# kieranrcampbell/clonealign

Hardware: AMD Instinct MI355X
Metric: ELBO iterations/sec (higher is better)
Workload: dtype f32 variables (contraction: float64 series over gene bins; count-matrix products: int8 MFMA, exact); 1 GPU; synthetic 100000 cells x 5000 genes x 8 clones, K=1, S=1, cell-sharded over 1 GPU(s) (BASELINE.json configs[2]); cells=100000, genes=5000, clones=8, K=1, mc_samples=1, y_storage=u8, y_bytes_per_elem=1, fused_sweep=True, fwd_mfma=True, series_form=True, y_mfma=True, parallelism=single, collective=none, allreduce_doubles_per_train_pass=20764, build_id=f943299e0af595e5

## Files before the change

### clonealign_amd/csrc/ca_eng_create.inc

```

constexpr double CA_ML_STREAM_FIXED_US = 6.6;
constexpr double CA_ML_STREAM_BYTES_PER_US = 5.62e6;
constexpr double CA_ML_MIN_STREAM_US = 45.0;
constexpr int CA_ML_MAX_PER = 4;
struct ca_mom_last_in {
  int slots;
  int n_cu;
  int nb_stream, nb_ovf;
  int ngrp, nred;
  int64_t image_bytes;
};
inline int ca_mom_last_free(const ca_mom_last_in& a) { return std::max(a.slots - a.nb_stream, 0); }
inline int ca_mom_last_free_x(const ca_mom_last_in& a) {
  const int xcd = std::max(a.n_cu / 32, 1);
  return a.slots / xcd - cdiv(a.nb_stream, xcd);
}
inline int ca_mom_last_per(const ca_mom_last_in& a) {
  const int xcd = std::max(a.n_cu / 32, 1), free_x = ca_mom_last_free_x(a);
  if (free_x < 1) return 0;
  return std::max(1, cdiv(a.ngrp, free_x * xcd));
}
inline bool ca_mom_last_pick(const ca_mom_last_in& a) {
  if (a.nb_stream + a.ngrp + a.nred <= a.slots) return false;
  const int per = ca_mom_last_per(a);
  if (per < 1 || per > CA_ML_MAX_PER) return false;
  return CA_ML_STREAM_FIXED_US + (double)a.image_bytes / CA_ML_STREAM_BYTES_PER_US >= CA_ML_MIN_STREAM_US;
}

int create_impl(ca_engine* h, const ca_problem* p) {
  const int N = (int)h->N; (void)N;
  HIPCK(h, hipSetDevice(h->device));
  hipDeviceProp_t prop;
  HIPCK(h, hipGetDeviceProperties(&prop, h->device));
  h->n_cu = prop.multiProcessorCount > 0 ? prop.multiProcessorCount : 256;
  HIPCK(h, hipStreamCreateWithFlags(&h->stream, hipStreamNonBlocking));
  HIPCK(h, hipStreamCreateWithFlags(&h->stream2, hipStreamNonBlocking));
  HIPCK(h, hipEventCreateWithFlags(&h->ev_params, hipEventDisableTiming));
  HIPCK(h, hipEventCreateWithFlags(&h->ev_ydone, hipEventDisableTiming));
  {
    int lo = 0, hi = 0;
    if (hipDeviceGetStreamPriorityRange(&lo, &hi) != hipSuccess) { (void)hipGetLastError(); lo = hi = 0; }
    if (hipStreamCreateWithPriority(&h->stream3, hipStreamNonBlocking, hi) != hipSuccess) { (void)hipGetLastError(); h->stream3 = nullptr; }
  }
  HIPCK(h, hipEventCreateWithFlags(&h->ev_poly0, hipEventDisableTiming));
  HIPCK(h, hipEventCreateWithFlags(&h->ev_poly1, hipEventDisableTiming));
  HIPCK(h, hipEventCreateWithFlags(&h->ev_ywdone, hipEventDisableTiming));
  h->async_y = variant_on(h, CA_VAR_ASYNC_Y, "CA_ASYNC_Y") &&
               ((double)h->N * (double)h->G >= 4e7 || variantx_on(h, CA_VARX_ASYNC_SMALL, "CA_ASYNC_SMALL"));
  HIPCK(h, hipHostMalloc((void**)&h->host_pinned, 64 * sizeof(double)));
  memset(h->host_pinned, 0, 64 * sizeof(double));
  if (hipHostGetDevicePointer((void**)&h->host_dev, h->host_pinned, 0) != hipSuccess) { h->host_dev = nullptr; (void)hipGetLastError(); }
  h->mon_tail = no_small_args();
  h->tail_fuse = variant_on(h, CA_VAR_TAIL_FUSE, "CA_TAIL_FUSE");
  h->pre_ok = variant_on(h, CA_VAR_PRE, "CA_PRE");
  h->upd_merge = h->tail_fuse && h->pre_ok && variant_on(h, CA_VAR_UPDATE_MERGE, "CA_UPDATE_MERGE");
  h->p2p_ride = h->tail_fuse && variant_on(h, CA_VAR_P2P_RIDE, "CA_P2P_RIDE");
  h->run_gate = h->upd_merge && variant_on(h, CA_VAR_RUN_GATE, "CA_RUN_GATE");
  {
    int khz = 0;
    if (hipDeviceGetAttribute(&khz, hipDeviceAttributeWallClockRate, h->device) == hipSuccess && khz >= 1000) h->ticks_per_us = (double)khz / 1000.0;
    else (void)hipGetLastError();
  }
  h->gate_ticks = (unsigned long long)(h->ticks_per_us * (double)(h->opt.gate_timeout_us > 0 ? h->opt.gate_timeout_us : 1000));
  h->run_fwd = h->run_gate && variantx_on(h, CA_VARX_RUN_FWD, "CA_RUN_FWD");
  h->pair_elbo = variant_on(h, CA_VAR_PAIR_ELBO, "CA_PAIR_ELBO");
  CACK(h->sp_in ? upload_y_sparse(h, p, h->sp_in) : upload_y(h, p));
  const int G = h->G, C = h->C, K = h->K, P = h->P, S = h->S, D = h->D;
  const int64_t Nn = h->N;
  h->nchunk = cdiv(C, CA_CW);
  h->ngblk = cdiv(G, CA_TB);
  {
    int CP = 1;
    while (CP < C) CP <<= 1;
    h->ncblk = (C <= 64) ? std::min(cdiv(Nn, CA_TB / CP), 16 * 256) : cdiv(Nn, CA_TB);
  }
  const int target_blocks = 8 * h->n_cu;
  const int nfb = cdiv(Nn, CA_TB * kFwdR);
  h->gsplit = std::max(1, std::min(std::min(target_blocks / std::max(nfb, 1), 16), std::max(1, G / 64)));
  h->gsplit = std::max(h->gsplit, cdiv(G, 1024));
  if (const int t = tune_val(h, CA_TUNE_GSPLIT, "CA_GSPLIT")) h->gsplit = std::max(std::max(1, t), cdiv(G, 1024));
  h->gchunk = cdiv(G, h->gsplit);
  h->gsplit = cdiv(G, h->gchunk);
  h->RG = G >= 1024 ? 4 : 1;
  if (const int r = tune_val(h, CA_TUNE_RG, "CA_RG")) { if (r == 1 || r == 4 || r == 8) h->RG = r; }
  h->ntile = cdiv(G, 64 * h->RG);
  const int gblocks = cdiv(h->ntile, CA_TB / 64);
  h->csplit = (int)std::max<int64_t>(1, std::min<int64_t>(cdiv(target_blocks, gblocks), std::max<int64_t>(1, Nn / 64)));
  if (const int t = tune_val(h, CA_TUNE_CSPLIT, "CA_CSPLIT")) h->csplit = std::max(1, t);
  h->cchunk = (Nn + h->csplit - 1) / h->csplit;
  h->csplit = cdiv(Nn, h->cchunk);
  h->TR = 128;
  const int tr_set = tune_val(h, CA_TUNE_TR, "CA_TR");
  if (tr_set) h->TR = std::min(128, std::max(1, tr_set));
  h->nrb = cdiv(Nn, h->TR);
  while (!tr_set && (int64_t)h->nrb * h->nseg < 4 * h->n_cu && h->TR > 32) { h->TR /= 2; h->nrb = cdiv(Nn, h->TR); }
  h->nrg = cdiv(h->nrb, CA_TB / 64);
  std::vector<double> Lrm((size_t)G * C), logL((size_t)G * C);
  std::vector<float> Lb((size_t)(h->nchunk + (h->nchunk & 1)) * G * CA_CW, 0.f);
  for (int g = 0; g < G; ++g)
    for (int c = 0; c < C; ++c) {
      const double v = p->L[hidx(p->layout, g, c, G, C)];
      Lrm[(size_t)g * C + c] = v;
      logL[(size_t)g * C + c] = std::log(v);
      Lb[((size_t)(c / CA_CW) * G + g) * CA_CW + (c % CA_CW)] = (float)v;
    }
  CACK(dalloc(h, &h->Lb, (int64_t)Lb.size()));
  CACK(upload_f(h, h->Lb, Lb));
  double* logL_dev = nullptr; double* extra_dev = nullptr;
  HIPCK(h, hipMalloc((void**)&logL_dev, logL.size() * sizeof(double)));
// ... 145 lines not shown
    }
    int zsplit = h->gsplit;
    if (h->fwd_mfma) {
      h->frow = 16;
      h->nk32 = cdiv(G, 32);
      const int cblocks = cdiv(Nn, (CA_TB / 64) * CA_FM_TL * 16);
      {
        int per_cu = 4;
        const void* fn = (D == 1) ? (const void*)k_fwd_mfma<1> : (const void*)k_fwd_mfma<2>;
        if (hipOccupancyMaxActiveBlocksPerMultiprocessor(&per_cu, fn, CA_TB, 0) != hipSuccess || per_cu < 1) per_cu = 4;
        (void)hipGetLastError();
        h->fsplit = pick_split(cblocks, (int64_t)per_cu * h->n_cu, std::max(1, std::min(16, h->nk32 / CA_FM_KC)), 0.02);
      }
      if (const int t = tune_val(h, CA_TUNE_FSPLIT, "CA_FSPLIT")) h->fsplit = std::max(1, std::min(t, h->nk32));
      h->fkchunk = cdiv(h->nk32, h->fsplit);
      h->fsplit = cdiv(h->nk32, h->fkchunk);
      zsplit = h->fsplit;
      CACK(dalloc(h, &h->Mq, (int64_t)h->nk32 * 2 * 64 * 8 * ((h->c16 || h->s2) ? 2 : 1)));
    } else {
      CACK(dalloc(h, &h->Mb2, (int64_t)G * h->frow));
    }
    CACK(dalloc(h, &h->mu32B, G));
    CACK(dalloc(h, &h->gene_partB, (int64_t)h->ngblk * (3 + K)));
    CACK(dalloc(h, &h->gene_part_alt, (int64_t)h->ngblk * (3 + K)));
    CACK(dalloc(h, &h->gene_partB_alt, (int64_t)h->ngblk * (3 + K)));
    if (!h->fwd_cell) CACK(dalloc(h, &h->Zpart2, (int64_t)zsplit * Nn * h->frow));
  }
  if (!h->fwd_cell) h->async_y = false;
  if (verbose(h))
    fprintf(stderr, "[clonealign_hip] N=%lld G=%d C=%d D=%d n_cu=%d gsplit=%d gchunk=%d csplit=%d fused=%d fwd_mfma=%d fsplit=%d fkchunk=%d "
            "bwd_mfma=%d csplit_m=%d cchunk_m=%lld nwt=%d fwd_cell=%d fc_tl=%d fc_nbig=%d ncblk_f=%d ystore=%d async_y=%d\n", (long long)Nn, G, C, D, h->n_cu, h->gsplit,
            h->gchunk, h->csplit, (int)h->fused_ok, (int)h->fwd_mfma, h->fsplit, h->fkchunk, (int)h->bwd_mfma, h->csplit_m,
            (long long)h->cchunk_m, h->nwt, (int)h->fwd_cell, h->fc_tl, h->fc_nbig, h->ncblk_f, h->ystore, (int)h->async_y);
  CACK(dalloc(h, &h->vmm, 2 * std::max(D, 1)));
  CACK(dalloc(h, &h->vmm_part, (int64_t)h->ngblk * 2 * std::max(D, 1)));
  CACK(dalloc(h, &h->etamax2, h->N16));
  CACK(dalloc(h, &h->gene_part, (int64_t)h->ngblk * (3 + K)));
  CACK(dalloc(h, &h->Zpart, (int64_t)S * h->gsplit * h->nchunk * Nn * CA_CW));
  CACK(dalloc(h, &h->coef, (int64_t)S * h->nchunk * Nn * CA_CW));
  CACK(dalloc(h, &h->scratch, Nn * C));
  const int64_t n_cpart = std::max(std::max(h->ncblk, h->ncblk_f), h->n_cu);
  CACK(dalloc(h, &h->cell_part, n_cpart * (3 + C)));
#ifdef CA_SERIES_ALWAYS
  const bool series_auto = true;
#else
  const bool series_auto = Nn >= 6000 && (double)G >= 2000.0 + (h->opt.world > 1 ? 7.5e7 : 2.5e7) / (double)Nn;
#endif
  h->adam_bound = ca_adam_step_bound(h->opt.learning_rate, h->opt.beta1, h->opt.beta2);
  h->poly_shape = ca_poly_ok(D, S, C) && h->fused_ok && !h->c16 && !h->s2 && K == 1 && h->adam_bound > 0 &&
                  (variant_on(h, CA_VAR_SERIES, "CA_SERIES") || variantx_on(h, CA_VARX_SERIES, "CA_SERIES_ON"));
  h->poly = h->poly_shape && ((series_auto && variant_on(h, CA_VAR_SERIES, "CA_SERIES")) || variantx_on(h, CA_VARX_SERIES, "CA_SERIES_ON"));
  if (h->poly) {
    int CPp = 1;
    while (CPp < C) CPp <<= 1;
    const int per_cu = (h->opt.reserved[0] >= 1 && h->opt.reserved[0] <= 8) ? h->opt.reserved[0] : 2;
    const int ncb = (int)std::min<int64_t>(cdiv(Nn, CA_TB / CPp), (int64_t)per_cu * h->n_cu);
    h->poly_side = h->opt.reserved[1] == 1;
    const size_t wb = ca_poly_workspace_bytes(G, ncb);
    CACK(dalloc(h, &h->poly_mem, (int64_t)wb));
    HIPCK(h, hipMemsetAsync(h->poly_mem, 0, wb, h->stream));
    ca_poly_bind(&h->pws, h->poly_mem, G, ncb);
    HIPCK(h, hipHostMalloc((void**)&h->poly_ring, 16 * 4 * sizeof(double), hipHostMallocMapped));
    memset(h->poly_ring, 0, 16 * 4 * sizeof(double));
    if (hipHostGetDevicePointer((void**)&h->poly_ring_dev, h->poly_ring, 0) != hipSuccess) { (void)hipGetLastError(); h->poly = false; }
    CACK(dalloc(h, &h->poly_xpart, cdiv(Nn, CA_TB)));
    CACK(dalloc(h, &h->poly_zero, Nn));
    HIPCK(h, hipMemsetAsync(h->poly_zero, 0, (size_t)Nn * sizeof(float), h->stream));
  }
  CACK(dalloc(h, &h->ee_partB, n_cpart));
  CACK(dalloc(h, &h->gpart, (int64_t)std::max(h->csplit, h->csplit_m) * G * (S + D)));
  CACK(dalloc(h, &h->dFpart, (int64_t)std::max(h->ntile, h->nwt) * Nn * std::max(D, 1)));
  CACK(dalloc(h, &h->YWpart, (int64_t)(h->nseg + 1) * Nn * std::max(K, 1)));
  CACK(dalloc(h, &h->YTpart, (int64_t)(h->nrb + 1) * h->Gp * std::max(K, 1)));
  CACK(dalloc(h, &h->YW, Nn * std::max(K, 1)));
  h->n_yw = cdiv(Nn, CA_TB);
  CACK(dalloc(h, &h->yw_part, h->n_yw));
  CACK(dalloc(h, &h->ytpsi, (int64_t)h->Gp * std::max(K, 1)));
  if (h->ystore == CA_YSTORE_U8 && K == 1 && h->Gp < (1 << 21) && Nn < ((int64_t)1 << 26) && variant_on(h, CA_VAR_Y_MFMA1, "CA_Y_MFMA1")) {
    h->ys_N64 = (Nn + 63) / 64 * 64;
    h->ys_nseg = h->Gp / CA_YS_GW;
    h->ys_RS = 64;
    while (h->ys_RS < 512 && cdiv(Nn, 4 * h->ys_RS) * h->ys_nseg > 4 * h->n_cu) h->ys_RS *= 2;
    h->ys_nrg = cdiv(Nn, 4 * h->ys_RS);
    const bool y4_force = variantx_on(h, CA_VARX_Y4, "CA_Y4_ON");
    if (variant_on(h, CA_VAR_Y4, "CA_Y4") && (h->poly || y4_force) && (double)Nn * (double)h->Gp < 2.0e9) {
      const int64_t nkeys = (int64_t)h->ys_nrg * h->ys_nseg * 4 * h->ys_RS;
      CACK(dalloc(h, &h->esc_off, nkeys + 1));
      const int64_t nw = Nn * h->ys_nseg;
      hipLaunchKernelGGL(k_esc_count, dim3(cdiv(nw * 64, CA_YM_TB)), dim3(CA_YM_TB), 0, h->stream, (const uint8_t*)h->Y, Nn, h->Gp, h->ys_nseg, h->ys_RS,
                         h->esc_off);
      hipLaunchKernelGGL(k_esc_scan, dim3(1), dim3(1024), 0, h->stream, h->esc_off, nkeys);
      HIPCK(h, hipGetLastError());
      int total = 0;
      HIPCK(h, hipMemcpyAsync(&total, h->esc_off + nkeys, sizeof(int), hipMemcpyDeviceToHost, h->stream));
      SYNC(h);
      h->n_esc = total;
      h->ys4 = h->n_esc * 256 <= Nn * (int64_t)h->G || y4_force;
      if (!h->ys4) {
        HIPCK(h, hipFree(h->esc_off));
        h->allocs.pop_back();
        h->dev_bytes -= 4 * (nkeys + 1);
        h->esc_off = nullptr;
      } else {
        CACK(dalloc(h, &h->esc, h->n_esc));
        hipLaunchKernelGGL(k_esc_fill, dim3(cdiv(nw * 64, CA_YM_TB)), dim3(CA_YM_TB), 0, h->stream, (const uint8_t*)h->Y, Nn, h->Gp, h->ys_nseg, h->ys_RS,
                           h->esc_off, h->esc);
        HIPCK(h, hipGetLastError());
      }
    }
    CACK(dalloc(h, &h->Ys, h->ys_N64 * h->Gp / (h->ys4 ? 2 : 1)));
    uint8_t *wr = nullptr, *pr = nullptr;
    CACK(dalloc(h, &wr, (int64_t)(h->Gp / 64) * 1024));
    CACK(dalloc(h, &pr, (h->ys_N64 / 64) * 1024));
    h->Wr = (uint4*)wr; h->Pr = (uint4*)pr;
    CACK(dalloc(h, &h->Wsum, (int64_t)(h->Gp / 64) * 4));
    CACK(dalloc(h, &h->Psum, (h->ys_N64 / 64) * 4));
    CACK(dalloc(h, &h->YWpart, (int64_t)(std::max(h->nseg, h->ys_nseg) + 1) * Nn));
    CACK(dalloc(h, &h->YTpart, (int64_t)(std::max(h->nrb, h->ys_nrg) + 1) * h->Gp));
    CACK(dalloc(h, &h->ys_exps, 6));
    CACK(dalloc(h, &h->ys_amax, 2));
    h->ys_nq = cdiv((int64_t)(h->Gp / 64) + h->ys_N64 / 64, CA_YM_TB / 64);
    h->ys_ncap = std::max(h->ys_nq, h->ngblk + cdiv(Nn, CA_TB)) + 2;
    CACK(dalloc(h, &h->ys_amaxp, (int64_t)3 * h->ys_ncap * 2));
    if (h->ys4)
      hipLaunchKernelGGL(k_pack_y4, dim3(cdiv(h->ys_N64 * (h->Gp / 32), CA_YM_TB)), dim3(CA_YM_TB), 0, h->stream, (const uint8_t*)h->Y, (uint4*)h->Ys, Nn,
                         h->ys_N64, h->Gp);
    else
      hipLaunchKernelGGL(k_bias_y, dim3(cdiv(h->ys_N64 * (h->Gp / 16), CA_YM_TB)), dim3(CA_YM_TB), 0, h->stream, (const uint8_t*)h->Y, (uint4*)h->Ys, Nn,
                         h->ys_N64, h->Gp);
    HIPCK(h, hipGetLastError());
    if (h->adam_bound > 0) h->ys_step_bound = (float)(1.02 * h->adam_bound);
    h->y_ys = true;
    h->y_dev_bytes += h->ys4 ? h->ys_N64 * h->Gp / 2 + 4 * h->n_esc + 4 * ((int64_t)h->ys_nrg * h->ys_nseg * 4 * h->ys_RS + 1) : h->ys_N64 * h->Gp;
  }
  h->mom_ride = h->poly && h->y_ys && !h->poly_side && h->host_dev && variant_on(h, CA_VAR_MOM_RIDE, "CA_MOM_RIDE");
  if (h->mom_ride) {
    ca_mom_last_in ml;
    int per_cu = 0;
    const hipError_t oe = h->ys4 ? (h->n_ovf > 0 ? hipOccupancyMaxActiveBlocksPerMultiprocessor(&per_cu, k_ys_mfma_ovf_mom<true>, CA_YM_TB, CA_YS4_LDS_BYTES)
                                                 : hipOccupancyMaxActiveBlocksPerMultiprocessor(&per_cu, k_ys_mfma_mom<true>, CA_YM_TB, CA_YS4_LDS_BYTES))
                                 : (h->n_ovf > 0 ? hipOccupancyMaxActiveBlocksPerMultiprocessor(&per_cu, k_ys_mfma_ovf_mom<false>, CA_YM_TB, CA_YS_LDS_BYTES)
                                                 : hipOccupancyMaxActiveBlocksPerMultiprocessor(&per_cu, k_ys_mfma_mom<false>, CA_YM_TB, CA_YS_LDS_BYTES));
    if (oe != hipSuccess) { (void)hipGetLastError(); per_cu = 0; }
    ml.slots = per_cu * h->n_cu; ml.n_cu = h->n_cu;
    ml.nb_stream = h->ys_nrg * h->ys_nseg;
    ml.nb_ovf = h->n_ovf > 0 ? cdiv(Nn, CA_TB) + cdiv(h->n_ovf_chunk, CA_TB / 64) : 0;
    ml.ngrp = h->pws.n_gene_blocks; ml.nred = CA_MOM_NRED;
    ml.image_bytes = h->ys_N64 * h->Gp / (h->ys4 ? 2 : 1);
    h->mom_free_slots = ca_mom_last_free(ml);
    h->mom_last = variantx_on(h, CA_VARX_MOM_LAST, "CA_MOM_LAST_ON") || (variant_on(h, CA_VAR_MOM_LAST, "CA_MOM_LAST") && ca_mom_last_pick(ml));
    if (h->opt.variant_off & CA_VAR_MOM_LAST) h->mom_last = false;
    if (h->mom_last) {
      const int per = ca_mom_last_per(ml);
      h->mom_per = per < 1 ? CA_MOM_PER : std::min(per, CA_ML_MAX_PER);
      h->mom_nred = 2 * CA_MOM_NRED;
      const int lab = (h->opt.reserved[1] & ~0xFF) ? h->opt.reserved[1] >> 8 : 0;
      if (lab & 15) h->mom_per = lab & 15;
      if (lab & 16) h->mom_nred = CA_MOM_NRED;
      h->mom_ovf_first = (lab & 32) != 0;
    }
  }
  h->cell_lean = h->poly && variant_on(h, CA_VAR_CELL_LEAN, "CA_CELL_LEAN");
  h->cell_mfma = h->poly && variant_on(h, CA_VAR_CELL_MFMA, "CA_CELL_MFMA");
  h->ride_ok = h->ystore == CA_YSTORE_U8 && K == 1 && D <= 2 && h->fused_ok && !h->c16 && h->fwd_cell && (h->fc_tl == 6 || h->fc_tl == 8 || (h->fc_tl == 2 && h->fc_nbig == 0)) &&
               !h->y_ys && variant_on(h, CA_VAR_Y_RIDE, "CA_Y_RIDE");
  const bool tl1_ok = h->fc_tl == 1 && h->fc_nbig == 0 && !h->c16;
  h->ride_ys = h->y_ys && (!h->ys4 || (h->poly && D == 1 && !h->c16 && !h->s2)) && D <= 2 && h->fused_ok && h->fwd_cell && (h->fc_tl == 6 || tl1_ok || (h->fc_tl == 2 && h->fc_nbig == 0)) &&
               variant_on(h, CA_VAR_Y_RIDE, "CA_Y_RIDE");
  h->yfin_split = h->ride_ys && h->bwd_mfma && h->tail_fuse && variant_on(h, CA_VAR_YFIN_RIDE, "CA_YFIN_RIDE");
  if (h->y_ys && !h->ride_ys) h->async_y = false;
  {
    const int tiles = cdiv(Nn, 16), qb = tiles / std::max(h->n_cu, 1), rb = tiles - qb * h->n_cu;
    h->fwd_bal = h->ride_ys && !h->c16 && !h->s2 && D == 1 && C <= 8 && qb >= 1 && qb <= 6 && h->nk32 >= 96 && h->host_dev && variant_on(h, CA_VAR_FWD_BAL, "CA_FWD_BAL");
    if (h->fwd_bal) {
      h->bal_q = qb; h->bal_r = rb;
      h->bal_nchunk = rb > 0 ? std::min(CA_BAL_MAXCHUNK, h->n_cu / rb) : 0;
      CACK(dalloc(h, &h->bal_xw, std::max<int64_t>(1, (int64_t)rb * h->bal_nchunk * 512)));
    }
  }
  h->s2f = h->s2 && h->fused_ok && h->fwd_cell && (h->fc_tl == 2 || h->fc_tl == 6) && (h->ride_ys || !h->ride_ok) && variant_on(h, CA_VAR_S2_FUSE, "CA_S2_FUSE");
  h->layout_series = h->poly || (h->poly_shape && h->opt.world > 1);
  if (h->layout_series) {
    h->off_y = 3 + C;
    h->off_q = h->off_y + (int64_t)h->Gp * K;
    h->off_x = h->off_q + (int64_t)CA_PL_NB * (CA_PL_R + 2) * 8;
    h->off_g = h->off_x + std::max(h->opt.world, 1);
    h->red_n = h->off_g + (int64_t)G * (S + D);
    CACK(dalloc(h, &h->red, h->red_n));
    if (h->poly) h->pws.tabQ = h->red + h->off_q;
  } else {
  h->off_g = 3 + C;
  h->off_y = h->off_g + (int64_t)G * (S + D);
  h->red_n = h->off_y + (int64_t)G * K;
  CACK(dalloc(h, &h->red, h->off_y + (int64_t)h->Gp * std::max(K, 1)));
  }
  CACK(dalloc(h, &h->terms_dev, 4));
  CACK(ensure_elbo_cap(h, 64));
  CACK(ensure_eps_cap(h, 1));
  {
    const int cols = 1 + ((K > 0) ? P : 0);
    const int cols_all = cols + (p->loc0 ? 0 : 1);
    std::vector<double> srow;
    if (!p->loc0) {
      srow.resize((size_t)Nn);
      HIPCK(h, hipMemcpyAsync(srow.data(), h->s64, (size_t)Nn * sizeof(double), hipMemcpyDeviceToHost, h->stream));
      SYNC(h);
    }
    std::vector<double> cs((size_t)G, 0.0), ytx((size_t)G * std::max(P, 1), 0.0);
    float *Ft = nullptr, *Vt = nullptr, *YWp = nullptr, *YTp = nullptr; double* yt = nullptr;
    HIPCK(h, hipMalloc((void**)&Ft, (size_t)Nn * sizeof(float)));
    HIPCK(h, hipMalloc((void**)&Vt, (size_t)G * sizeof(float)));
    HIPCK(h, hipMalloc((void**)&YWp, (size_t)h->nseg * Nn * sizeof(float)));
    HIPCK(h, hipMalloc((void**)&YTp, (size_t)h->nrb * h->Gp * sizeof(float)));
// ... 66 lines not shown
```

### clonealign_amd/csrc/ca_eng_loop.inc

```
int wait_y(ca_engine* h, bool all) {
  if (all) {
    if (h->y_pending) HIPCK(h, hipStreamWaitEvent(h->stream, h->ev_ydone, 0));
    h->y_pending = false; h->yw_pending = false;
  } else if (h->yw_pending) {
    HIPCK(h, hipStreamWaitEvent(h->stream, h->ev_ywdone, 0));
    h->yw_pending = false;
  }
  return CA_OK;
}

int make_etamax(ca_engine* h) {
  if (h->D > 0) {
    LAUNCH(h, CA_KERNEL_OTHER, hipLaunchKernelGGL(k_vmm_final, dim3(1), dim3(64), 0, h->stream, h->vmm_part, h->vmm, h->ngblk, h->D));
    LAUNCH(h, CA_KERNEL_OTHER, hipLaunchKernelGGL(k_etamax, dim3(cdiv(h->N, CA_TB)), dim3(CA_TB), 0, h->stream, h->F, h->vmm, h->etamax2, h->N, h->D));
  }
  h->em_stale = false;
  return CA_OK;
}
int ensure_etamax(ca_engine* h) {
  if (!h->em_stale) return CA_OK;
  return make_etamax(h);
}

int refresh_derived(ca_engine* h) {
  CACK(wait_y(h, true));
  h->y_defer = false;
  h->pre_valid = false;
  h->ys_steps = -1;
  h->ys_quant_ready = false;
  if (h->D > 0) LAUNCH(h, CA_KERNEL_OTHER, hipLaunchKernelGGL(k_vprep, dim3(h->ngblk), dim3(CA_TB), 0, h->stream, h->V, h->Vs, h->vmm_part, h->G, h->D));
  CACK(make_etamax(h));
  h->gaux_slot = -1;
  h->ycache_valid = false;
  h->yfin_pending = false;
  h->look_valid = false;
  h->poly_fresh = false;
  h->poly_seq_base = h->poly_seq + 1;
  h->poly_xmax_ready = false;
  h->poly_xglob_steps = -1;
  return CA_OK;
}

ca_ovf_args ovf_args(ca_engine* h, float* YWextra) {
  ca_ovf_args ovf;
  memset(&ovf, 0, sizeof(ovf));
  if (h->n_ovf > 0) {
    ovf.nb_rows = cdiv(h->N, CA_TB); ovf.nb_chunks = cdiv(h->n_ovf_chunk, CA_TB / 64);
    ovf.rowptr = h->ovf_rowptr; ovf.col = h->ovf_col; ovf.val = h->ovf_val; ovf.YWextra = YWextra;
    ovf.chunk_start = h->ovf_chunk_start; ovf.row2 = h->ovf_row2; ovf.val2 = h->ovf_val2; ovf.csum = h->ovf_csum; ovf.nchunk = h->n_ovf_chunk;
  }
  return ovf;
}
ca_yfin_args yfin_args(ca_engine* h, int rows, int nseg) {
  ca_yfin_args a;
  memset(&a, 0, sizeof(a));
  a.ncol = cdiv((int64_t)h->Gp * h->K, 64); a.nrow = h->n_yw;
  a.part = h->YTpart; a.out = h->red + h->off_y; a.rows = rows; a.ld = (int64_t)h->Gp * h->K; a.cols = h->Gp * h->K; a.G = h->G;
  if (h->n_ovf > 0) { a.col_chunk_ptr = h->ovf_col_chunk_ptr; a.csum = h->ovf_csum; }
  a.YWpart = h->YWpart; a.nseg = nseg + (h->n_ovf > 0 ? 1 : 0); a.F = h->F; a.D = h->D; a.N = h->N; a.YW = h->YW; a.yw_part = h->yw_part;
  return a;
}
int launch_yfinish(ca_engine* h, int rows, int nseg) {
  const ca_yfin_args a = yfin_args(h, rows, nseg);
  LAUNCH(h, CA_KERNEL_OTHER, hipLaunchKernelGGL(k_yfinish, dim3(a.ncol + a.nrow), dim3(1024), 0, h->stream, a.part, a.out, a.rows, a.ld, a.cols, a.col_chunk_ptr,
                                                a.csum, h->K, a.G, a.ncol, a.YWpart, a.nseg, a.F, a.D, a.N, a.YW, a.yw_part));
  return CA_OK;
}

ca_ysq_args ys_quant_args(ca_engine* h, int steps, bool* lagged) {
  ca_ysq_args a;
  memset(&a, 0, sizeof(a));
  const int s0 = h->ys_slot, s1 = (s0 + 1) % 3;
  a.nblk = h->ys_nq;
  a.V = h->V; a.Dv = h->D; a.G = h->G; a.GS = h->Gp / 64; a.F = h->F; a.Df = h->D; a.N = h->N; a.NS = h->ys_N64 / 64;
  *lagged = steps >= 0 && steps <= 4 && h->ys_step_bound > 0.f;
  if (*lagged) {
    a.amax_in = h->ys_amaxp + (int64_t)s0 * h->ys_ncap * 2; a.n_in = h->ys_namax[s0];
    a.slack_w = a.slack_p = (float)steps * h->ys_step_bound;
  } else {
    a.amax_in = reinterpret_cast<const float*>(h->ys_amax); a.n_in = 1;
  }
  a.amax_out = h->ys_amaxp + (int64_t)s1 * h->ys_ncap * 2;
  h->ys_namax[s1] = h->ys_nq;
  a.exps = h->ys_exps + 2 * s0; a.Wr = h->Wr; a.Pr = h->Pr; a.Wsum = h->Wsum; a.Psum = h->Psum;
  return a;
}
int ys_quant(ca_engine* h) {
  if (h->ys_quant_ready) return CA_OK;
  bool lagged = false;
  ca_ysq_args a = ys_quant_args(h, h->ys_steps, &lagged);
  if (!lagged) {
    HIPCK(h, hipMemsetAsync(h->ys_amax, 0, 2 * sizeof(unsigned), h->stream));
    LAUNCH(h, CA_KERNEL_OTHER, hipLaunchKernelGGL(k_ym_absmax, dim3(cdiv(std::max<int64_t>(h->N, h->G), CA_YM_TB)), dim3(CA_YM_TB), 0, h->stream,
                                                  h->V, h->D, (int64_t)h->G, h->F, h->D, h->N, 1, h->ys_amax));
  }
  LAUNCH(h, CA_KERNEL_OTHER, hipLaunchKernelGGL(k_ys_quant, dim3(a.nblk), dim3(CA_YM_TB), 0, h->stream, a));
  return CA_OK;
}
ca_ys_io ys_io(ca_engine* h) {
  ca_ys_io io;
  io.Wr = h->Wr; io.Pr = h->Pr; io.Wsum = h->Wsum; io.Psum = h->Psum; io.exps = h->ys_exps + 2 * h->ys_slot;
  io.YWpart = h->YWpart; io.YTpart = h->YTpart;
  io.esc_off = h->ys4 ? h->esc_off : nullptr; io.esc = h->ys4 ? h->esc : nullptr;
  return io;
}
ca_ovf_args ys_ovf(ca_engine* h) { return ovf_args(h, h->YWpart + (int64_t)h->ys_nseg * h->N); }
int yfin_flush(ca_engine* h) {
  if (!h->yfin_pending) return CA_OK;
  h->yfin_pending = false;
  return launch_yfinish(h, h->ys_nrg, h->ys_nseg);
}
int ys_finish(ca_engine* h, bool defer = false) {
  h->yfin_pending = true;
  if (!defer) CACK(yfin_flush(h));
  h->ys_slot = (h->ys_slot + 1) % 3;
  h->ys_steps = 0;
  h->ys_quant_ready = false;
  h->ycache_valid = true;
  return CA_OK;
}
template <bool Y4>
void launch_ys(ca_engine* h) {
  constexpr int lds = Y4 ? CA_YS4_LDS_BYTES : CA_YS_LDS_BYTES;
  const int nb_main = h->ys_nrg * h->ys_nseg;
  const ca_pm_args* pm = h->mom_args;
  h->mom_args = nullptr;
  const int nmom = pm ? pm->nmb + pm->nred : 0;
  if (h->n_ovf > 0) {
    const ca_ovf_args ovf = ys_ovf(h);
    const dim3 grid(nmom + nb_main + ovf.nb_rows + ovf.nb_chunks);
    if (pm) {
      ca_pm_args pmo = *pm;
      if (h->mom_last && h->mom_ovf_first) pmo.blk0 += ovf.nb_rows + ovf.nb_chunks;
      hipLaunchKernelGGL(k_ys_mfma_ovf_mom<Y4>, grid, dim3(CA_YM_TB), lds, h->stream, h->Ys, ys_io(h), h->N, h->Gp, h->ys_RS, nb_main, ovf, h->F, h->V, h->D, pmo);
    }
    else hipLaunchKernelGGL(k_ys_mfma_ovf<Y4>, grid, dim3(CA_YM_TB), lds, h->stream, h->Ys, ys_io(h), h->N, h->Gp, h->ys_RS, nb_main, ovf, h->F, h->V, h->D);
  } else {
    if (pm) hipLaunchKernelGGL(k_ys_mfma_mom<Y4>, dim3(nmom + nb_main), dim3(CA_YM_TB), lds, h->stream, h->Ys, ys_io(h), h->N, h->Gp, h->ys_RS, *pm);
    else hipLaunchKernelGGL(k_ys_mfma<Y4>, dim3(nb_main), dim3(CA_YM_TB), lds, h->stream, h->Ys, ys_io(h), h->N, h->Gp, h->ys_RS);
  }
}
int ycache_ys(ca_engine* h) {
  CACK(ys_quant(h));
  if (h->ys4) LAUNCH(h, CA_KERNEL_YPASS, launch_ys<true>(h));
  else LAUNCH(h, CA_KERNEL_YPASS, launch_ys<false>(h));
  const bool defer = h->ys_defer_next;
  h->ys_defer_next = false;
  return ys_finish(h, defer);
}

int ensure_ycache(ca_engine* h) {
  if (h->y_defer) {
    h->y_defer = false;
    HIPCK(h, hipStreamWaitEvent(h->stream2, h->ev_params, 0));
    std::swap(h->stream, h->stream2);
    h->on_side = true;
    const int rc = ensure_ycache(h);
    h->on_side = false;
    std::swap(h->stream, h->stream2);
    CACK(rc);
    HIPCK(h, hipEventRecord(h->ev_ydone, h->stream2));
    h->y_pending = true;
    HIPCK(h, hipEventRecord(h->ev_ywdone, h->stream2));
    h->yw_pending = true;
    return CA_OK;
  }
  if (h->ycache_valid || h->K == 0) { h->ycache_valid = true; return yfin_flush(h); }
  h->yfin_pending = false;
  if (h->y_ys) return ycache_ys(h);
  dim3 grid((unsigned)((int64_t)h->nrg * h->nseg));
  const ca_ovf_args ovf = ovf_args(h, h->YWpart + (int64_t)h->nseg * h->N * h->K);
  ca_ovf_args none;
  memset(&none, 0, sizeof(none));
  const ca_ypass_ops fit = {h->F, h->D, h->V, h->YWpart, h->YTpart, h->K};
  for (int koff = 0; koff < h->K; koff += 4) {
    const int kk = std::min(4, h->K - koff);
    CACK(prof_begin(h, CA_KERNEL_YPASS));
    const ca_ovf_args& o = koff == 0 ? ovf : none;
    ypass<0>(h, fit, koff, kk, grid, o);
    HIPCK(h, hipGetLastError());
    CACK(prof_end(h));
  }
  if (!h->on_side) {
    CACK(launch_yfinish(h, h->nrg, h->nseg));
  } else {
    LAUNCH(h, CA_KERNEL_OTHER, hipLaunchKernelGGL(k_colsum, dim3(cdiv((int64_t)h->Gp * h->K, 64)), dim3(1024), 0, h->stream,
                                                  h->YTpart, h->red + h->off_y, h->nrg, (int64_t)h->Gp * h->K, h->Gp * h->K,
                                                  h->n_ovf > 0 ? h->ovf_col_chunk_ptr : nullptr, h->n_ovf > 0 ? h->ovf_csum : nullptr, h->K, h->G));
    LAUNCH(h, CA_KERNEL_OTHER, hipLaunchKernelGGL(k_yw_dot, dim3(h->n_yw), dim3(CA_TB), 0, h->stream, h->YWpart,
                                                  h->nseg + (h->n_ovf > 0 ? 1 : 0), h->F, h->D, h->K, h->N, h->YW, h->yw_part));
  }
  h->ycache_valid = true;
  return CA_OK;
}


ca_small_args small_args(ca_engine* h, const double* gene_part, int apply, float lr_t, double* elbo_dst, bool reduce_cells) {
  ca_small_args a;
  a.enabled = 1;
  a.red = h->red; a.gene_part = gene_part; a.ngblk = h->ngblk;
  a.vchi = h->vchi; a.alpha_u = h->alpha_u; a.m_v = h->m_v; a.v_v = h->v_v; a.m_a = h->m_a; a.v_a = h->v_a; a.g_v = h->g_v; a.g_a = h->g_a;
  a.elbo_out = elbo_dst; a.terms_out = h->terms_dev;
  a.G = h->G; a.C = h->C; a.K = h->K; a.apply = apply;
  a.lr_t = lr_t; a.b1 = (float)h->opt.beta1; a.b2 = (float)h->opt.beta2; a.aeps = (float)h->opt.adam_eps;
  a.vmm_part = h->vmm_part; a.vmm = h->vmm; a.D = h->D;
  a.dir_const = h->dir_const;
  a.cell_part = reduce_cells ? h->cell_part : nullptr; a.ncblk = h->ncblk;
  a.host_out = nullptr; a.host_flag = nullptr; a.host_seq = 0; a.reduce_only = 0;
  a.yw_part = nullptr; a.n_yw = 0;
  a.ee_part = nullptr; a.n_ee = 0;
  a.vchi_out = nullptr; a.alpha_out = nullptr;
  if (!apply && elbo_dst && h->host_seq_next && h->host_dev) {
    a.host_out = h->host_dev + 32;
    a.host_flag = reinterpret_cast<unsigned long long*>(h->host_dev + 33);
    a.host_seq = h->host_seq_next;
    h->host_seq_next = 0;
  }
  return a;
}
int mon_tail_local_sums(ca_engine* h) {
  if (!h->mon_tail.enabled || !h->mon_tail.cell_part) return CA_OK;
  CACK(wait_y(h, false));
  ca_small_args r = h->mon_tail;
  r.reduce_only = 1; r.host_out = nullptr;
  LAUNCH(h, CA_KERNEL_OTHER, hipLaunchKernelGGL(k_final_small, dim3(1), dim3(CA_TB), 0, h->stream, r));
  h->mon_tail.cell_part = nullptr; h->mon_tail.yw_part = nullptr;
  return CA_OK;
// ... 753 lines not shown
```

### clonealign_amd/csrc/ca_eng_state.inc

```
namespace {

thread_local std::string g_last_error;

typedef struct { char internal[128]; } ca_nccl_uid;
typedef void* ca_nccl_comm;
struct RcclApi {
  void* lib = nullptr;
  int (*GetUniqueId)(ca_nccl_uid*) = nullptr;
  int (*CommInitRank)(ca_nccl_comm*, int, ca_nccl_uid, int) = nullptr;
  int (*CommDestroy)(ca_nccl_comm) = nullptr;
  int (*AllReduce)(const void*, void*, size_t, int, int, ca_nccl_comm, hipStream_t) = nullptr;
  const char* (*GetErrorString)(int) = nullptr;
  std::string err;
  bool load() {
    if (lib) return true;
    const char* cands[] = {getenv("CLONEALIGN_RCCL_LIB"), "librccl.so.1", "librccl.so", "/opt/rocm/lib/librccl.so.1",
                           "/opt/rocm/lib/librccl.so"};
    for (const char* c : cands) {
      if (!c || !*c) continue;
      lib = dlopen(c, RTLD_NOW | RTLD_LOCAL);
      if (lib) break;
    }
    if (!lib) { err = std::string("cannot dlopen librccl: ") + dlerror(); return false; }
    GetUniqueId = (decltype(GetUniqueId))dlsym(lib, "ncclGetUniqueId");
// ... 64 lines not shown
  const ca_sparse* sp_in = nullptr;
  float* Lb = nullptr;
  double *A = nullptr, *cn = nullptr, *s64 = nullptr, *colsum = nullptr, *YtX = nullptr;
  float* s32 = nullptr;
  float *F = nullptr, *m_psi = nullptr, *v_psi = nullptr;
  float *glogit = nullptr, *m_gl = nullptr, *v_gl = nullptr;
  float *V = nullptr, *m_V = nullptr, *v_V = nullptr;
  float *loc = nullptr, *ls = nullptr, *m_loc = nullptr, *v_loc = nullptr, *m_ls = nullptr, *v_ls = nullptr;
  float* loc_init = nullptr;
  float *vchi = nullptr, *m_v = nullptr, *v_v = nullptr;
  float *alpha_u = nullptr, *m_a = nullptr, *v_a = nullptr;
  float *vchi_alt = nullptr, *alpha_u_alt = nullptr;
  bool upd_merge = false, em_stale = false;
  bool run_gate = false, gate_req = false, gate_armed = false;
  unsigned long long gate_ticks = 100000ull; std::chrono::steady_clock::time_point gate_t0;
  double ticks_per_us = 100.0;
  bool gate_open = false, gate_aborted = false, in_run = false; struct gate_snapshot* gate_snap = nullptr; struct fwd_snapshot* gate_fsnap = nullptr;
  bool run_fwd = false;
  bool fwd_gate = false;
  unsigned long long gate_seq = 0; unsigned long long* gate_local = nullptr;
  bool p2p_ride = false;
  double* gaux = nullptr; int64_t gaux_slot = -1;
  int gaux_idx = 0;
  int* vmm_at = nullptr; int vmm_at_idx = 0; bool vmm_at_ready = false;
  double dir_const = 0.0;
  float b1p = 0.f, b2p = 0.f;
  float *g_loc = nullptr, *g_ls = nullptr, *g_V = nullptr, *g_v = nullptr, *g_a = nullptr, *g_psi = nullptr, *dgl = nullptr;
  float* eps_dev = nullptr; int64_t eps_cap = 0;
  float *mu32 = nullptr, *Mb = nullptr, *Vs = nullptr, *vmm = nullptr, *vmm_part = nullptr, *etamax2 = nullptr;
  double* gene_part = nullptr; int ngblk = 0;
  float *Zpart = nullptr, *coef = nullptr; double* scratch = nullptr;
  double* cell_part = nullptr; int ncblk = 0;
  float *gpart = nullptr, *dFpart = nullptr; int gsplit = 1, gchunk = 0, csplit = 1; int64_t cchunk = 0; int RG = 4, ntile = 0;
  float *YWpart = nullptr, *YTpart = nullptr, *YW = nullptr; double* ytpsi = nullptr;
  double* red = nullptr; int64_t red_n = 0, off_g = 0, off_y = 0;
  int64_t off_q = 0, off_x = 0;
  bool poly_shape = false, layout_series = false;
  bool mon_tail_local = false;
  bool poly_xslot_pending = false;
  int poly_xglob_steps = -1;
  double* elbo_dev = nullptr; int64_t elbo_cap = 0; double* terms_dev = nullptr;
  double* host_pinned = nullptr;
  bool ycache_valid = false, sums_global = false, sums_started = false;
  std::vector<double> mu_part;
  bool fused_ok = false, look_valid = false; int64_t look_slot = 0; int frow = 8;
  bool carry = false, carry_builtin = false; std::vector<float> carry_eps;
  int64_t n_series = 0, n_series_fallback = 0;
  double *poly_ring = nullptr, *poly_ring_dev = nullptr; uint64_t poly_seq = 0, poly_seq_base = 1, adam_steps = 0, poly_steps_at[16] = {};
  bool mom_ride = false; unsigned mom_tag = 0; const ca_pm_args* mom_args = nullptr;
  bool mom_last = false, mom_ovf_first = false; int mom_free_slots = 0, mom_per = CA_MOM_PER, mom_nred = CA_MOM_NRED;
  bool cell_mfma = false;
  bool cell_lean = false;
  bool poly = false, poly_side = false, poly_y_defer = false, poly_fresh = false, poly_df = false ; ca_poly_ws pws; float* poly_zero = nullptr; unsigned char* poly_mem = nullptr;
  float *Mb2 = nullptr, *mu32B = nullptr, *Zpart2 = nullptr; double* gene_partB = nullptr;
  bool y_defer = false;
  bool ride_ok = false;
  bool ride_ys = false;
  bool fold_gsum = false, fold_now = false;
  int64_t hint_A = -1, hint_B = -1, pre_A = -1, pre_B = -1;
  bool pre_valid = false, pre_ok = true, pair_elbo = true;
  double* ee_partB = nullptr;
  double *gene_part_alt = nullptr, *gene_partB_alt = nullptr;
  bool bwd_ready = false; int64_t bwd_slot = -1;
  double* yw_part = nullptr; int n_yw = 0;
  bool yfin_split = false, yfin_pending = false;
  ca_small_args mon_tail;
  bool tail_fuse = true;
  double* host_dev = nullptr;
  unsigned long long host_seq = 0, host_seq_next = 0;
  float* eps_stage = nullptr; size_t eps_stage_bytes = 0;
  hipEvent_t ev_stage = nullptr;
  bool fwd_cell = false; int ncblk_f = 0, fc_tl = 4;
  int fc_nbig = 0;
  bool fwd_mfma = false; int fsplit = 1, fkchunk = 1, nk32 = 1; unsigned short* Mq = nullptr;
  bool fwd_bal = false; int bal_q = 0, bal_r = 0, bal_nchunk = 0; unsigned long long* bal_xw = nullptr; unsigned bal_tag = 0;
  bool pfwd = false; int pf_npair = 0, pf_fsplit = 1, pf_kchunk = 1; unsigned short* pf_Mq = nullptr; float* pf_Z = nullptr;
  int bwd_pairs = 0;
  bool bwd_mfma = false, bwd_frac = false, c16 = false, s2 = false, s2f = false;
  unsigned short* coefq = nullptr; int64_t N16 = 0, cchunk_m = 0; int csplit_m = 1, nwt = 0;
  int bwd_tl = CA_BWD_TL;
  uint64_t draw = 0;
  hipEvent_t ev_ywdone = nullptr; bool yw_pending = false, on_side = false;
  bool y_ys = false, ys4 = false; int* esc_off = nullptr; unsigned* esc = nullptr; int64_t n_esc = 0;
  uint8_t* Ys = nullptr; uint4 *Wr = nullptr, *Pr = nullptr; int *Wsum = nullptr, *Psum = nullptr;
  int* ys_exps = nullptr;
  unsigned* ys_amax = nullptr;
  float* ys_amaxp = nullptr; int ys_nq = 0;
  int ys_ncap = 0, ys_namax[3] = {0, 0, 0};
  bool ys_quant_ready = false;
  int ys_slot = 0, ys_steps = -1, ys_RS = 256, ys_nrg = 0, ys_nseg = 0; int64_t ys_N64 = 0; float ys_step_bound = -1.f;
  double adam_bound = -1.0;
  ca_p2p* p2p = nullptr;
  ca_nccl_comm comm = nullptr;
  ca_host_allreduce_fn host_ar = nullptr; void* host_ar_user = nullptr; double* host_ar_buf = nullptr; int64_t host_ar_cap = 0;
  std::vector<EvPair> ev_pool; size_t ev_used = 0; bool prof_open = false;
  unsigned prof_seen[CA_KERNEL_COUNT] = {0, 0, 0, 0, 0};
  double k_ms[CA_KERNEL_COUNT] = {0}; int64_t k_n[CA_KERNEL_COUNT] = {0};
  int n_cu = 256;
};

namespace {

#define HIPCK(h, call)                                                                       \
  do {                                                                                       \
    hipError_t e_ = (call);                                                                  \
    if (e_ != hipSuccess) {                                                                  \
      (h)->err = std::string(#call) + ": " + hipGetErrorString(e_);                          \
      return CA_ERR_HIP;                                                                     \
    }                                                                                        \
  } while (0)

#define CACK(call)                \
  do {                            \
    int rc_ = (call);             \
    if (rc_ != CA_OK) return rc_; \
  } while (0)

int comm_check(ca_engine* h) {
  if (h->host_pinned && *reinterpret_cast<volatile unsigned int*>(h->host_pinned + 41) != 0u) {
    h->err = "a forward-sweep block gave up waiting for a chunk of a left-over tile (k_fwd_bal_ys); the engine's state is undefined";
    return CA_ERR_STATE;
  }
  if (h->host_pinned && *reinterpret_cast<volatile unsigned int*>(h->host_pinned + 43) != 0u) {
    h->err = "a reducer block of the series form's moment role gave up waiting for the moment blocks of its launch (k_ys_mfma_mom); the engine's state is undefined";
    return CA_ERR_STATE;
  }
  if (h->host_pinned && *reinterpret_cast<volatile unsigned int*>(h->host_pinned + 42) != 0u) {
    h->err = "the series form of the contraction (CA_VARX_SERIES) cannot cover this fit's exponent range: max|psi| (max W - min W) exceeds 4 x " +
             std::to_string(CA_PL_NB) + " bins' worth; the passes since are truncated -- start over without the series form";
    return CA_ERR_STATE;
  }
  if (h->p2p && h->p2p->err_host && *reinterpret_cast<volatile unsigned long long*>(h->p2p->err_host) != 0ull) {
    h->err = "peer-to-peer all-reduce #" + std::to_string(*reinterpret_cast<volatile unsigned long long*>(h->p2p->err_host)) +
             ": a peer's data did not arrive within the time limit (peer lost or out of step); this engine's transport is dead -- "
             "destroy the engine and start over in a fresh process";
    return CA_ERR_COMM;
  }
  return CA_OK;
}
#define SYNC(h)                                          \
  do {                                                   \
    HIPCK(h, hipStreamSynchronize((h)->stream));         \
    CACK(comm_check(h));                                 \
  } while (0)

template <typename T>
int dalloc(ca_engine* h, T** p, int64_t n) {
  if (n <= 0) n = 1;
  void* q = nullptr;
  hipError_t e = hipMalloc(&q, (size_t)n * sizeof(T));
  if (e != hipSuccess) {
    h->err = std::string("hipMalloc of ") + std::to_string(n * sizeof(T)) + " bytes: " + hipGetErrorString(e);
    return CA_ERR_NOMEM;
  }
  e = hipMemsetAsync(q, 0, (size_t)n * sizeof(T), h->stream);
  if (e == hipSuccess) e = hipStreamSynchronize(h->stream);
  if (e != hipSuccess) { h->err = hipGetErrorString(e); return CA_ERR_HIP; }
  h->allocs.push_back(q);
  h->dev_bytes += n * (int64_t)sizeof(T);
  *p = (T*)q;
  return CA_OK;
}

int prof_flush(ca_engine* h) {
  if (h->ev_used == 0) return CA_OK;
  SYNC(h);
// ... 227 lines not shown
```

### clonealign_amd/csrc/ca_kernels.hip.h

```cpp
#pragma once
#include <hip/hip_runtime.h>
#include <stdint.h>

#define CA_CW 8
#define CA_LOG2E_F 1.44269504088896340736f
#define CA_LN2 0.69314718055994530942
#define CA_LOG2PI 1.83787706640934548356
#define CA_TB 256

template <int CTRL, int ROW_MASK>
__device__ __forceinline__ float ca_dpp_pull(float v) {
  return __builtin_bit_cast(
      float, __builtin_amdgcn_update_dpp(0, __builtin_bit_cast(int, v), CTRL, ROW_MASK, 0xF, false));
}
__device__ __forceinline__ float ca_wave_sum_lane63(float v) {
  v += ca_dpp_pull<0xB1, 0xF>(v);
  v += ca_dpp_pull<0x4E, 0xF>(v);
  v += ca_dpp_pull<0x141, 0xF>(v);
  v += ca_dpp_pull<0x140, 0xF>(v);
  v += ca_dpp_pull<0x142, 0xA>(v);
  v += ca_dpp_pull<0x143, 0xC>(v);
  return v;
}

// ... 594 lines not shown
}

struct ca_p2p_args {
  double* const* peers;
  int rank, world;
  int64_t cap;
  unsigned long long seq;
  unsigned long long* err;
  unsigned int* err_local;
  unsigned long long timeout_ticks;
  const float* gpart; int nslice; int64_t fold_lo, fold_n;
  const double* yw_part; int n_yw; int64_t yw_index;
};
__device__ __forceinline__ unsigned long long* ca_p2p_entry(double* slab, int64_t cap, int world, int par, int src, int64_t i) {
  return reinterpret_cast<unsigned long long*>(slab) + 2 * ((((int64_t)par * world + src) * cap) + i);
}
#ifndef CA_P2P_LAB
#define CA_P2P_LAB 0
#endif
__global__ void __launch_bounds__(CA_TB) k_p2p_allreduce(double* __restrict__ buf, int64_t n, ca_p2p_args a) {
  __shared__ unsigned int bad;
  if (threadIdx.x == 0) bad = __hip_atomic_load(a.err_local, __ATOMIC_RELAXED, __HIP_MEMORY_SCOPE_AGENT) != 0u;
  __syncthreads();
  if (bad) return;
  const int par = (int)(a.seq & 1ull);
  const unsigned long long tag = (a.seq & 0xFFFFFFFFull) << 32;
  const int64_t i0 = (int64_t)blockIdx.x * CA_TB + threadIdx.x, stride = (int64_t)gridDim.x * CA_TB;
  double yw_sum = 0.0;
  if (a.yw_part && a.yw_index >= 0 && a.yw_index < n && (a.yw_index / CA_TB) % gridDim.x == blockIdx.x) {
    __shared__ double smy[CA_TB];
    double ya = 0.0;
    for (int b = threadIdx.x; b < a.n_yw; b += CA_TB) ya += a.yw_part[b];
    yw_sum = ca_block_sum(ya, smy);
  }
  double* mine = a.peers[a.rank];
  for (int64_t i = i0; i < n; i += stride) {
    double v;
    if (a.gpart && i >= a.fold_lo && i < a.fold_lo + a.fold_n) {
      v = 0.0;
      const float* gp = a.gpart + (i - a.fold_lo);
      for (int sp0 = 0; sp0 < a.nslice; sp0 += 8) {
        float t[8];
#pragma unroll
        for (int q = 0; q < 8; ++q) t[q] = gp[(int64_t)(sp0 + q < a.nslice ? sp0 + q : a.nslice - 1) * a.fold_n];
#pragma unroll
        for (int q = 0; q < 8; ++q) v += (sp0 + q < a.nslice) ? (double)t[q] : 0.0;
      }
    } else {
      v = buf[i];
    }
    if (a.yw_part && i == a.yw_index) v += yw_sum;
    const unsigned long long bits = (unsigned long long)__double_as_longlong(v);
    const unsigned long long w0 = (bits & 0xFFFFFFFFull) | tag, w1 = (bits >> 32) | tag;
    for (int p = 0; p < a.world; ++p) {
      unsigned long long* e = ca_p2p_entry(a.peers[p], a.cap, a.world, par, a.rank, i);
      __hip_atomic_store(e, w0, __ATOMIC_RELAXED, __HIP_MEMORY_SCOPE_SYSTEM);
      __hip_atomic_store(e + 1, w1, __ATOMIC_RELAXED, __HIP_MEMORY_SCOPE_SYSTEM);
    }
  }
  const unsigned long long t0 = __builtin_amdgcn_s_memrealtime();
  for (int64_t i = i0; i < n; i += stride) {
    double s = 0.0;
    for (int r = 0; r < a.world; ++r) {
      const unsigned long long* e = ca_p2p_entry(mine, a.cap, a.world, par, r, i);
      unsigned long long w0 = __hip_atomic_load(e, __ATOMIC_RELAXED, __HIP_MEMORY_SCOPE_SYSTEM);
      unsigned long long w1 = __hip_atomic_load(e + 1, __ATOMIC_RELAXED, __HIP_MEMORY_SCOPE_SYSTEM);
      while (((w0 ^ tag) >> 32) != 0ull || ((w1 ^ tag) >> 32) != 0ull) {
        if (__builtin_amdgcn_s_memrealtime() - t0 > a.timeout_ticks) {
          unsigned long long expect = 0ull;
          __hip_atomic_compare_exchange_strong(a.err, &expect, a.seq, __ATOMIC_RELAXED, __ATOMIC_RELAXED, __HIP_MEMORY_SCOPE_SYSTEM);
          __hip_atomic_store(a.err_local, 1u, __ATOMIC_RELAXED, __HIP_MEMORY_SCOPE_AGENT);
          return;
        }
        __builtin_amdgcn_s_sleep(1);
        w0 = __hip_atomic_load(e, __ATOMIC_RELAXED, __HIP_MEMORY_SCOPE_SYSTEM);
        w1 = __hip_atomic_load(e + 1, __ATOMIC_RELAXED, __HIP_MEMORY_SCOPE_SYSTEM);
      }
      s += __longlong_as_double((long long)((w0 & 0xFFFFFFFFull) | (w1 << 32)));
    }
    buf[i] = s;
  }
}

template <bool Y4>
__global__ void __launch_bounds__(CA_YM_TB, Y4 ? CA_YS4_WAVES : CA_YS_WAVES) k_ys_mfma_ovf(const uint8_t* __restrict__ Ys, ca_ys_io io, int64_t N, int Gp, int RS,
                                                                       int nb_main, ca_ovf_args ovf, const float* __restrict__ F,
                                                                       const float* __restrict__ V, int Dstride) {
  if ((int)blockIdx.x >= nb_main) {
    const int b = (int)blockIdx.x - nb_main;
    if (b < ovf.nb_rows) ca_ovf_rows_body(b, ovf.rowptr, ovf.col, ovf.val, V, Dstride, ovf.YWextra, N, 1, 0);
    else ca_ovf_chunks_body(b - ovf.nb_rows, ovf.chunk_start, ovf.row2, ovf.val2, F, Dstride, ovf.csum, ovf.nchunk, 1, 0);
    return;
  }
  extern __shared__ __attribute__((aligned(16))) unsigned char ca_ys_dyn[];
  ca_ys_mfma_body<Y4 ? CA_YS4_DEPTH : CA_YS_DEPTH, Y4, true>((int)blockIdx.x, Ys, io, N, Gp, RS, ca_ys_dyn);
}

#include "ca_polymom.hip.h"
static_assert(sizeof(ca_pm_lds) <= (size_t)CA_YS_LDS_BYTES && sizeof(ca_pm_lds) <= (size_t)CA_YS4_LDS_BYTES, "the moment role's tables fit the stream's dynamic LDS");
template <bool Y4>
__global__ void __launch_bounds__(CA_YM_TB, Y4 ? CA_YS4_WAVES : CA_YS_WAVES) k_ys_mfma_mom(const uint8_t* __restrict__ Ys, ca_ys_io io, int64_t N, int Gp, int RS, ca_pm_args pm) {
  extern __shared__ __attribute__((aligned(16))) unsigned char ca_ys_dyn[];
  const int nmom = pm.nmb + pm.nred, rb = (int)blockIdx.x - pm.blk0;
  if (rb >= 0 && rb < nmom) { ca_pm_ride_block<CA_YM_TB>(pm, rb, ca_ys_dyn); return; }
  ca_ys_mfma_body<Y4 ? CA_YS4_DEPTH : CA_YS_DEPTH, Y4, true>(rb < 0 ? (int)blockIdx.x : (int)blockIdx.x - nmom, Ys, io, N, Gp, RS, ca_ys_dyn);
}
template <bool Y4>
__global__ void __launch_bounds__(CA_YM_TB, Y4 ? CA_YS4_WAVES : CA_YS_WAVES) k_ys_mfma_ovf_mom(const uint8_t* __restrict__ Ys, ca_ys_io io, int64_t N, int Gp, int RS,
                                                                           int nb_main, ca_ovf_args ovf, const float* __restrict__ F,
                                                                           const float* __restrict__ V, int Dstride, ca_pm_args pm) {
  extern __shared__ __attribute__((aligned(16))) unsigned char ca_ys_dyn[];
  const int nmom = pm.nmb + pm.nred, rb = (int)blockIdx.x - pm.blk0;
  if (rb >= 0 && rb < nmom) { ca_pm_ride_block<CA_YM_TB>(pm, rb, ca_ys_dyn); return; }
  const int blk = rb < 0 ? (int)blockIdx.x : (int)blockIdx.x - nmom;
  if (blk >= nb_main) {
    const int b = blk - nb_main;
    if (b < ovf.nb_rows) ca_ovf_rows_body(b, ovf.rowptr, ovf.col, ovf.val, V, Dstride, ovf.YWextra, N, 1, 0);
    else ca_ovf_chunks_body(b - ovf.nb_rows, ovf.chunk_start, ovf.row2, ovf.val2, F, Dstride, ovf.csum, ovf.nchunk, 1, 0);
    return;
  }
  ca_ys_mfma_body<Y4 ? CA_YS4_DEPTH : CA_YS_DEPTH, Y4, true>(blk, Ys, io, N, Gp, RS, ca_ys_dyn);
}

struct ca_ysride_args {
  const uint8_t* Ys; ca_ys_io io;
  const float* F; const float* V; int Df;
  int Gp, RS, nb_main, nb_y;
  int pat_a, pat_b;
  int pers;
  ca_ovf_args ovf;
};
#ifndef CA_YS_RIDE_WAVES
#define CA_YS_RIDE_WAVES 4
#endif
template <int D, int TLB, int TLS, int DEPTH, bool C16 = false, bool S2F = false, bool Y4 = false>
__global__ void __launch_bounds__(CA_TB, (DEPTH == 1 && !C16 && !S2F) ? CA_YS_RIDE_WAVES : 3) k_fwd_cell_mix_ys(const float* __restrict__ F, const float* __restrict__ etamax2,
                                                           const float* __restrict__ Vs, const unsigned short* __restrict__ Mq,
                                                           ca_cell_ptrs p, const float* __restrict__ alpha_u,
                                                           double* __restrict__ cell_part, int64_t N, int C, int K, int nk, int nbig,
                                                           int nf, ca_ysride_args y) {
  constexpr size_t FW = sizeof(ca_f32x4) * 4 * TLB * 64 + sizeof(double) * (CA_TB + 64);
  constexpr size_t SM = FW > (size_t)CA_YS_LDS_BYTES ? FW : (size_t)CA_YS_LDS_BYTES;
  __shared__ __attribute__((aligned(16))) unsigned char smem[SM];
  if (p.gate) {
    if (*p.gate != p.gate_go) return;
  }
  int idx;
  bool sweep;
  if (y.pers > 0) {
    const int b = (int)blockIdx.x;
    sweep = b >= y.pers && b < y.pers + nf;
    idx = sweep ? b - y.pers : (b < y.pers ? b : y.nb_main + (b - y.pers - nf));
  } else {
    sweep = ca_ride_split((int)blockIdx.x, nf, y.nb_y, y.pat_a, y.pat_b, idx);
  }
  CA_LAB_BLOCK_T0();
#define CA_YS_LEAVE() CA_LAB_LEAVE(ca_ys_out)
  if (!sweep) {
    if (idx >= y.nb_main) {
      const int b = idx - y.nb_main;
      if (b < y.ovf.nb_rows) ca_ovf_rows_body(b, y.ovf.rowptr, y.ovf.col, y.ovf.val, y.V, y.Df, y.ovf.YWextra, N, 1, 0);
      else ca_ovf_chunks_body(b - y.ovf.nb_rows, y.ovf.chunk_start, y.ovf.row2, y.ovf.val2, y.F, y.Df, y.ovf.csum, y.ovf.nchunk, 1, 0);
      CA_YS_LEAVE();
    }
    CA_PRIO_STREAM();
    if (y.pers > 0) {
      for (int u = idx; u < y.nb_main; u += y.pers) {
        if (u != idx) __syncthreads();
        ca_ys_mfma_body<DEPTH, Y4>(u, y.Ys, y.io, N, y.Gp, y.RS, smem);
      }
    } else {
      ca_ys_mfma_body<DEPTH, Y4>(idx, y.Ys, y.io, N, y.Gp, y.RS, smem);
    }
    CA_YS_LEAVE();
  }
  {
    ca_f32x4* comb = reinterpret_cast<ca_f32x4*>(smem);
    double* sm = reinterpret_cast<double*>(smem + sizeof(ca_f32x4) * 4 * TLB * 64);
    double* la = sm + CA_TB;
    ca_log_softmax_alpha(alpha_u, C, la);
    if (nbig > 0 && idx >= nbig)
      ca_fwd_cell_body<D, TLS, C16, S2F>(F, etamax2, Vs, Mq, p, cell_part, N, C, K, nk, (int64_t)nbig * (TLB * 16) + (int64_t)(idx - nbig) * (TLS * 16), idx, comb, sm, la);
    else
      ca_fwd_cell_body<D, TLB, C16, S2F>(F, etamax2, Vs, Mq, p, cell_part, N, C, K, nk, (int64_t)idx * (TLB * 16), idx, comb, sm, la);
  }
#undef CA_YS_LEAVE
  CA_LAB_LABEL(ca_ys_out);
  CA_LAB_BLOCK_END(sweep ? (nbig > 0 && idx >= nbig ? 2 : 1) : 0, idx);
}

#include "ca_fwdbal.hip.h"
#include "ca_k_mse.hip.h"
#include "ca_k_loglik.hip.h"
#include "ca_k_blockll.hip.h"
#include "ca_k_pairll.hip.h"
#include "ca_k_dmll.hip.h"
#include "ca_k_project.hip.h"
#include "ca_k_simulate.hip.h"
#include "ca_k_predictive.hip.h"
#include "ca_k_logexpr.hip.h"
```

### clonealign_amd/csrc/ca_ymfma.hip.h

```cpp
#pragma once
#include <hip/hip_runtime.h>
#include <stdint.h>

typedef int ca_i32x4 __attribute__((ext_vector_type(4)));

#define CA_YM_TB 256

__device__ __forceinline__ int ca_fix_exp(float amax) { return amax > 0.f ? 29 - ilogbf(amax) : 0; }

__global__ void __launch_bounds__(CA_YM_TB) k_ym_absmax(const float* __restrict__ V, int Dv, int64_t G, const float* __restrict__ F, int Df,
                                                        int64_t N, int K, unsigned* __restrict__ amax) {
  const int64_t i = (int64_t)blockIdx.x * CA_YM_TB + threadIdx.x;
  float mw = 0.f, mp = 0.f;
  if (i < G) for (int k = 0; k < K; ++k) mw = fmaxf(mw, fabsf(V[i * Dv + k]));
  if (i < N) for (int k = 0; k < K; ++k) mp = fmaxf(mp, fabsf(F[i * Df + k]));
#pragma unroll
  for (int o = 32; o > 0; o >>= 1) { mw = fmaxf(mw, __shfl_xor(mw, o, 64)); mp = fmaxf(mp, __shfl_xor(mp, o, 64)); }
  if ((threadIdx.x & 63) == 0) {
    if (i < G + 64) atomicMax(amax, __float_as_uint(mw));
    if (i < N + 64) atomicMax(amax + 1, __float_as_uint(mp));
  }
}
__device__ __forceinline__ int ca_digit(int x, int p) {
  int d = 0;
#pragma unroll
  for (int i = 0; i <= 3; ++i) {
    d = (int)(signed char)(x & 0xFF);
    if (i == p) break;
    x = (x - d) >> 8;
  }
  return d;
}
__global__ void __launch_bounds__(CA_YM_TB) k_bias_y(const uint8_t* __restrict__ Y, uint4* __restrict__ Ys, int64_t N, int64_t N64, int Gp) {
  const int64_t i = (int64_t)blockIdx.x * CA_YM_TB + threadIdx.x;
  const int64_t per_piece = 256, nb = Gp / 64;
  if (i >= (N64 / 64) * nb * per_piece) return;
  const int c = (int)(i & 3), r = (int)((i >> 2) & 63);
  const int64_t piece = i >> 8;
  const int64_t cs = piece / nb, gb = piece - cs * nb;
  const int64_t n = cs * 64 + r;
  uint4 v = {0u, 0u, 0u, 0u};
  if (n < N) v = *reinterpret_cast<const uint4*>(Y + n * (int64_t)Gp + gb * 64 + 16 * c);
  v.x ^= 0x80808080u; v.y ^= 0x80808080u; v.z ^= 0x80808080u; v.w ^= 0x80808080u;
  Ys[i] = v;
}

__device__ __forceinline__ unsigned ca_nib4(unsigned lo, unsigned hi) {
  unsigned r = 0;
#pragma unroll
  for (int b = 0; b < 4; ++b) {
    const unsigned x = (lo >> (8 * b)) & 0xFFu, y = (hi >> (8 * b)) & 0xFFu;
    r |= ((x < 15u ? x : 15u) | ((y < 15u ? y : 15u) << 4)) << (8 * b);
  }
  return r;
}
__global__ void __launch_bounds__(CA_YM_TB) k_pack_y4(const uint8_t* __restrict__ Y, uint4* __restrict__ Y4, int64_t N, int64_t N64, int Gp) {
  const int64_t i = (int64_t)blockIdx.x * CA_YM_TB + threadIdx.x;
  const int64_t nb = Gp / 64;
  if (i >= (N64 / 64) * nb * 128) return;
  const int l = (int)(i & 63), ld = (int)((i >> 6) & 1);
  const int64_t piece = i >> 7, cs = piece / nb, gb = piece - cs * nb;
  const int64_t n0 = cs * 64 + 32 * ld + (l & 15), n1 = n0 + 16;
  const uint8_t* base = Y + gb * 64 + 16 * (l >> 4);
  uint4 a = {0u, 0u, 0u, 0u}, b = {0u, 0u, 0u, 0u};
  if (n0 < N) a = *reinterpret_cast<const uint4*>(base + n0 * (int64_t)Gp);
  if (n1 < N) b = *reinterpret_cast<const uint4*>(base + n1 * (int64_t)Gp);
  Y4[i] = (uint4){ca_nib4(a.x, b.x), ca_nib4(a.y, b.y), ca_nib4(a.z, b.z), ca_nib4(a.w, b.w)};
}
__device__ __forceinline__ int64_t ca_esc_key(int64_t n, int seg, int nseg, int RS) {
  const int64_t s = n / RS;
  return (((s >> 2) * nseg + seg) * 4 + (s & 3)) * RS + (n - s * RS);
}
__device__ __forceinline__ int ca_esc_count8(uint2 v) {
  int c = 0;
#pragma unroll
  for (int b = 0; b < 4; ++b) c += (((v.x >> (8 * b)) & 0xFFu) >= 15u) + (((v.y >> (8 * b)) & 0xFFu) >= 15u);
  return c;
}
__global__ void __launch_bounds__(CA_YM_TB) k_esc_count(const uint8_t* __restrict__ Y, int64_t N, int Gp, int nseg, int RS, int* __restrict__ off) {
  const int64_t w = ((int64_t)blockIdx.x * CA_YM_TB + threadIdx.x) >> 6;
  const int lane = threadIdx.x & 63;
  if (w >= N * nseg) return;
  const int64_t n = w / nseg;
  const int seg = (int)(w - n * nseg);
  int c = ca_esc_count8(*reinterpret_cast<const uint2*>(Y + n * (int64_t)Gp + seg * 512 + 8 * lane));
#pragma unroll
  for (int o = 32; o > 0; o >>= 1) c += __shfl_xor(c, o, 64);
  if (lane == 0) off[ca_esc_key(n, seg, nseg, RS)] = c;
}
__global__ void __launch_bounds__(1024) k_esc_scan(int* __restrict__ off, int64_t n) {
  __shared__ int64_t sm[1024];
  const int t = threadIdx.x;
  const int64_t chunk = (n + 1023) / 1024, a = t * chunk, b = (a + chunk < n) ? a + chunk : n;
  int64_t s = 0;
  for (int64_t i = a; i < b; ++i) s += off[i];
  sm[t] = s;
  __syncthreads();
  for (int o = 1; o < 1024; o <<= 1) {
    const int64_t v = t >= o ? sm[t - o] : 0;
    __syncthreads();
    sm[t] += v;
    __syncthreads();
  }
  int64_t run = sm[t] - s;
  for (int64_t i = a; i < b; ++i) { const int c = off[i]; off[i] = (int)run; run += c; }
  if (t == 1023) off[n] = (int)sm[1023];
}
__global__ void __launch_bounds__(CA_YM_TB) k_esc_fill(const uint8_t* __restrict__ Y, int64_t N, int Gp, int nseg, int RS, const int* __restrict__ off,
                                                       unsigned* __restrict__ esc) {
  const int64_t w = ((int64_t)blockIdx.x * CA_YM_TB + threadIdx.x) >> 6;
  const int lane = threadIdx.x & 63;
  if (w >= N * nseg) return;
  const int64_t n = w / nseg;
  const int seg = (int)(w - n * nseg);
  const uint2 v = *reinterpret_cast<const uint2*>(Y + n * (int64_t)Gp + seg * 512 + 8 * lane);
  const int c = ca_esc_count8(v);
  int x = c;
#pragma unroll
  for (int o = 1; o < 64; o <<= 1) { const int u = __shfl_up(x, o, 64); if (lane >= o) x += u; }
  int e = off[ca_esc_key(n, seg, nseg, RS)] + x - c;
  const unsigned cl = (unsigned)(n % RS);
#pragma unroll
  for (int b = 0; b < 8; ++b) {
    const unsigned y = ((b < 4 ? v.x : v.y) >> (8 * (b & 3))) & 0xFFu;
    if (y >= 15u) esc[e++] = cl | ((unsigned)(8 * lane + b) << 9) | ((y - 15u) << 18);
  }
}

__device__ __forceinline__ ca_i32x4 ca_mfma_i8(uint4 a, uint4 b, ca_i32x4 c) {
  return __builtin_amdgcn_mfma_i32_16x16x64_i8(__builtin_bit_cast(ca_i32x4, a), __builtin_bit_cast(ca_i32x4, b), c, 0, 0, 0);
}

constexpr int CA_YS_GW = 512;
static_assert(CA_YS_GW == 512, "k_ys_mfma's accumulator switch has eight cases");
constexpr int CA_YS_PITCH = 80;

__device__ __forceinline__ void ca_ds_read_tr_b8_x8(unsigned addr, uint2 (&lo)[4], uint2 (&hi)[4]) {
  asm volatile(
      "ds_read_b64_tr_b8 %0, %8\n\tds_read_b64_tr_b8 %4, %8 offset:640\n\t"
      "ds_read_b64_tr_b8 %1, %8 offset:16\n\tds_read_b64_tr_b8 %5, %8 offset:656\n\t"
      "ds_read_b64_tr_b8 %2, %8 offset:32\n\tds_read_b64_tr_b8 %6, %8 offset:672\n\t"
      "ds_read_b64_tr_b8 %3, %8 offset:48\n\tds_read_b64_tr_b8 %7, %8 offset:688\n\t"
      "s_waitcnt lgkmcnt(0)"
      : "=&v"(lo[0]), "=&v"(lo[1]), "=&v"(lo[2]), "=&v"(lo[3]), "=&v"(hi[0]), "=&v"(hi[1]), "=&v"(hi[2]), "=&v"(hi[3])
      : "v"(addr)
      : "memory");
}
__device__ __forceinline__ void ca_ds_read_tr_b8_x4(unsigned addr, uint2 (&lo)[2], uint2 (&hi)[2]) {
  asm volatile(
      "ds_read_b64_tr_b8 %0, %4\n\tds_read_b64_tr_b8 %2, %4 offset:640\n\t"
      "ds_read_b64_tr_b8 %1, %4 offset:16\n\tds_read_b64_tr_b8 %3, %4 offset:656\n\t"
      "s_waitcnt lgkmcnt(0)"
      : "=&v"(lo[0]), "=&v"(lo[1]), "=&v"(hi[0]), "=&v"(hi[1])
      : "v"(addr)
      : "memory");
}
static_assert(8 * CA_YS_PITCH == 640, "offsets in ca_ds_read_tr_b8_x8 / _x4 assume the 80-byte pitch");
__device__ __forceinline__ uint4 ca_and4(uint4 a, unsigned m) { return (uint4){a.x & m, a.y & m, a.z & m, a.w & m}; }

#ifndef CA_YS_DEPTH
#define CA_YS_DEPTH 2
#endif
#ifndef CA_YS_WAVES
#define CA_YS_WAVES 3
#endif
struct ca_ys_io {
  const uint4* Wr; const uint4* Pr; const int* Wsum; const int* Psum; const int* exps;
  float* YWpart; float* YTpart;
  const int* esc_off; const unsigned* esc;
};
#ifndef CA_YS4_DEPTH
#define CA_YS4_DEPTH 4
#endif
#ifndef CA_YS4_WAVES
#define CA_YS4_WAVES 4
#endif
constexpr int CA_YS4_OFF_W = 4 * 64 * CA_YS_PITCH;
constexpr int CA_YS4_OFF_ROW = CA_YS4_OFF_W + (CA_YS_GW / 64) * 1024;
constexpr int CA_YS4_OFF_PSI = CA_YS4_OFF_ROW + 4 * 64 * 8;
constexpr int CA_YS4_OFF_COL = 4 * (CA_YS_GW / 64) * 64 * 4 * 4;
constexpr int CA_YS4_LDS_BYTES = CA_YS4_OFF_COL + CA_YS_GW * 8;
static_assert(CA_YS4_OFF_PSI + 4 * 256 <= CA_YS4_OFF_COL, "the 4-bit launch's tables fit below its column-escape sums");
static_assert(4 * CA_YS4_LDS_BYTES <= 160 * 1024, "four blocks of the 4-bit launch per CU");
template <int DEPTH = CA_YS_DEPTH, bool Y4 = false, bool OWN = false>
__device__ __forceinline__ void ca_ys_mfma_body(int blk, const uint8_t* __restrict__ Ys, const ca_ys_io& io, int64_t N, int Gp,
                                                int RS ,
                                                unsigned char* ca_ys_lds ) {
  const uint4* __restrict__ Wr = io.Wr;
  const uint4* __restrict__ Pr = io.Pr;
  constexpr bool Y4L = Y4 && OWN;
  constexpr int NP = CA_YS_GW / 64;
  static_assert(NP % DEPTH == 0, "pieces per cell step must be a multiple of the pipeline depth");
  const int lane = threadIdx.x & 63, j = lane & 15, q = lane >> 4;
  const int wv = __builtin_amdgcn_readfirstlane((int)(threadIdx.x >> 6) & 3);
  const int nseg = Gp / CA_YS_GW;
  const int rg = blk / nseg, seg = blk - rg * nseg;
  unsigned char* my = ca_ys_lds + (size_t)wv * 64 * CA_YS_PITCH;
  const int64_t c0 = ((int64_t)rg * 4 + wv) * RS;
  const int64_t c1 = (c0 + RS < N) ? c0 + RS : N;
  const int g0 = seg * CA_YS_GW;
  const unsigned grp = (unsigned)(j >> 2);
  unsigned msk[4];
#pragma unroll
  for (int t = 0; t < 4; ++t) msk[t] = grp == (unsigned)t ? 0xFFFFFFFFu : 0u;
  ca_i32x4 acc_yt[NP];
#pragma unroll
  for (int a = 0; a < NP; ++a) acc_yt[a] = (ca_i32x4){0, 0, 0, 0};
  const int lrow = lane >> 2, lch = lane & 3;
  unsigned char* wr_dst = my + lrow * CA_YS_PITCH + 16 * lch;
  const unsigned char* rd_row = my + j * CA_YS_PITCH + 16 * q;
  const unsigned rd_tr = (unsigned)(size_t)my + (unsigned)((16 * q + (j >> 1)) * CA_YS_PITCH + 8 * (j & 1));
  constexpr int PB = Y4 ? 2048 : 4096, NL = PB / 1024;
  const uint8_t* src = Ys + ((c0 >> 6) * (int64_t)(Gp / 64) + (g0 >> 6)) * PB;
  const uint4* wsrc = Wr + (int64_t)(g0 >> 6) * 64;
  const unsigned voff = 16u * (unsigned)lane;
  uint4 R[DEPTH][NL], W[DEPTH];
  const int nsteps = c0 < c1 ? (int)((c1 - c0 + 63) / 64) : 0;
  typedef unsigned ca_v4u __attribute__((ext_vector_type(4)));
  const __amdgpu_buffer_rsrc_t ry = __builtin_amdgcn_make_buffer_rsrc(const_cast<uint8_t*>(src), 0, 0x7FFFFFFF, 0x00020000);
  const __amdgpu_buffer_rsrc_t rw = __builtin_amdgcn_make_buffer_rsrc(const_cast<uint4*>(wsrc), 0, NP * 1024, 0x00020000);
  const __amdgpu_buffer_rsrc_t rp = __builtin_amdgcn_make_buffer_rsrc(const_cast<uint4*>(Pr + (c0 >> 6) * 64), 0, 0x7FFFFFFF, 0x00020000);
  auto issue = [&](int slot, int st, int a, unsigned vo) {
    const int so = (st * (Gp / 64) + a) * PB;
#pragma unroll
    for (int i = 0; i < NL; ++i) {
      const ca_v4u v = __builtin_amdgcn_raw_buffer_load_b128(ry, (int)(vo + 1024u * (unsigned)i), so, 2 );
      R[slot][i] = (uint4){v.x, v.y, v.z, v.w};
    }
    if (!Y4L) {
      const ca_v4u w = __builtin_amdgcn_raw_buffer_load_b128(rw, (int)voff, a * 1024, 0);
      W[slot] = (uint4){w.x, w.y, w.z, w.w};
    }
  };
  uint4* wl = reinterpret_cast<uint4*>(ca_ys_lds + CA_YS4_OFF_W);
  unsigned long long* colesc = reinterpret_cast<unsigned long long*>(ca_ys_lds + CA_YS4_OFF_COL);
  uint4 wimg[2];
  int eoff = 0;
  if (Y4L) {
    wimg[0] = wsrc[threadIdx.x];
    wimg[1] = wsrc[threadIdx.x + CA_YM_TB];
    if (lane <= nsteps) eoff = io.esc_off[((int64_t)blk * 4 + wv) * RS + (64 * lane < RS ? 64 * lane : RS)];
  }
  uint4 pr_nx = {0u, 0u, 0u, 0u};
  if (nsteps > 0) {
    if (Y4L) {
      const ca_v4u pv = __builtin_amdgcn_raw_buffer_load_b128(rp, (int)voff, 0, 0);
      pr_nx = (uint4){pv.x, pv.y, pv.z, pv.w};
    }
#pragma unroll
    for (int d_ = 0; d_ < DEPTH; ++d_) issue(d_, 0, d_, voff);
  }
  if (Y4L) {
    static_assert(2 * CA_YM_TB == CA_YS_GW, "the block's threads hold the segment's W image and column sums in two halves");
    wl[threadIdx.x] = wimg[0];
    wl[threadIdx.x + CA_YM_TB] = wimg[1];
    colesc[threadIdx.x] = 0ull;
    colesc[threadIdx.x + CA_YM_TB] = 0ull;
    __syncthreads();
  }
  ca_i32x4 acc_yw[4];
  uint4 prm[4];
  int wtot[4] = {0, 0, 0, 0};
  if (!Y4) {
    const int* ws = io.Wsum + (g0 >> 6) * 4;
#pragma unroll
    for (int a = 0; a < NP; ++a)
#pragma unroll
      for (int p_ = 0; p_ < 4; ++p_) wtot[p_] += ws[a * 4 + p_];
  }
  const int e_w = io.exps[0];
  const int64_t kb = ((int64_t)blk * 4 + wv) * RS;
  unsigned long long* rowesc = reinterpret_cast<unsigned long long*>(ca_ys_lds + (Y4L ? CA_YS4_OFF_ROW : 4 * 64 * CA_YS_PITCH)) + wv * 64;
  unsigned char* psl = ca_ys_lds + CA_YS4_OFF_PSI + wv * 256;
  if (Y4) rowesc[lane] = 0ull;
  for (int st = 0; st < nsteps; ++st) {
    const int64_t cs = c0 + (int64_t)st * 64;
    const bool more = st + 1 < nsteps;
    uint4 pr;
    if (Y4L) {
      pr = pr_nx;
#pragma unroll
      for (int t = 0; t < 4; ++t) acc_yw[t] = (ca_i32x4){0, 0, 0, 0};
    } else {
      const ca_v4u pv = __builtin_amdgcn_raw_buffer_load_b128(rp, (int)voff, st * 1024, 0);
      pr = (uint4){pv.x, pv.y, pv.z, pv.w};
#pragma unroll
      for (int t = 0; t < 4; ++t) { acc_yw[t] = (ca_i32x4){0, 0, 0, 0}; if (!Y4L) prm[t] = ca_and4(pr, msk[t]); }
    }
    int e_lo = 0, e_hi = 0;
    unsigned en0 = 0u, en1 = 0u;
    if (Y4L) {
      e_lo = __builtin_amdgcn_readlane(eoff, st);
      e_hi = __builtin_amdgcn_readlane(eoff, st + 1);
      if (e_hi > e_lo) {
        en0 = io.esc[e_lo + lane < e_hi ? e_lo + lane : e_hi - 1];
        en1 = io.esc[e_lo + 64 + lane < e_hi ? e_lo + 64 + lane : e_hi - 1];
      }
    }
#pragma unroll
    for (int a = 0; a < NP; ++a) {
      const int slot = a % DEPTH;
      __builtin_amdgcn_sched_barrier(0);
      const uint4 wr = Y4L ? wl[a * 64 + lane] : W[slot];
      if (Y4) {
#pragma unroll
        for (int t = 0; t < 4; ++t) {
          const uint4 v = R[slot][t >> 1];
          const int sh = 4 * (t & 1);
          const uint4 av = ca_and4((uint4){v.x >> sh, v.y >> sh, v.z >> sh, v.w >> sh}, 0x0F0F0F0Fu);
          *reinterpret_cast<uint4*>(const_cast<unsigned char*>(rd_row) + 16 * t * CA_YS_PITCH) = av;
          acc_yw[t] = ca_mfma_i8(av, wr, acc_yw[t]);
        }
        if (a + DEPTH < NP) issue(slot, st, a + DEPTH, voff);
        else if (Y4L) {
          const unsigned vo = more ? voff : 0x80000000u + voff;
          if (a + DEPTH == NP) {
            const ca_v4u pv = __builtin_amdgcn_raw_buffer_load_b128(rp, (int)vo, (st + 1) * 1024, 0);
            pr_nx = (uint4){pv.x, pv.y, pv.z, pv.w};
          }
          issue(slot, st + 1, a + DEPTH - NP, vo);
        } else if (more) issue(slot, st + 1, a + DEPTH - NP, voff);
      } else {
#pragma unroll
        for (int i = 0; i < 4; ++i) *reinterpret_cast<uint4*>(wr_dst + 16 * i * CA_YS_PITCH) = R[slot][i];
        if (a + DEPTH < NP) issue(slot, st, a + DEPTH, voff);
        else if (more) issue(slot, st + 1, a + DEPTH - NP, voff);
#pragma unroll
        for (int t = 0; t < 4; ++t) {
          const uint4 av = *reinterpret_cast<const uint4*>(rd_row + 16 * t * CA_YS_PITCH);
          acc_yw[t] = ca_mfma_i8(av, wr, acc_yw[t]);
        }
      }
#pragma unroll
      for (int h2 = 0; h2 < 2; ++h2) {
        uint2 lo[2], hi[2];
        ca_ds_read_tr_b8_x4(rd_tr + 32u * (unsigned)h2, lo, hi);
#pragma unroll
        for (int t = 0; t < 2; ++t) {
          uint4 pa;
          if (Y4L) {
            unsigned g_ = grp;
            asm volatile("" : "+v"(g_));
            pa = ca_and4(pr, g_ == (unsigned)(2 * h2 + t) ? 0xFFFFFFFFu : 0u);
          } else {
            pa = prm[2 * h2 + t];
          }
          acc_yt[a] = ca_mfma_i8(pa, (uint4){lo[t].x, lo[t].y, hi[t].x, hi[t].y}, acc_yt[a]);
        }
      }
    }
    if (Y4L) {
      if (j < 4) *reinterpret_cast<uint4*>(psl + (4 * q + j) * 16) = pr;
      const unsigned char* wlb = reinterpret_cast<const unsigned char*>(wl);
      auto esc1 = [&](unsigned en) {
        const int c = (int)(en & 63u), gi = (int)((en >> 9) & 511u);
        const unsigned char* dw = wlb + ((gi >> 6) * 64 + 16 * ((gi >> 4) & 3)) * 16 + (gi & 15);
        const unsigned char* dp = psl + 64 * (c >> 4) + (c & 15);
        unsigned fw = 0u, fp = 0u;
#pragma unroll
        for (int p_ = 0; p_ < 4; ++p_) {
          fw += (unsigned)(int)(signed char)dw[16 * p_] << (8 * p_);
          fp += (unsigned)(int)(signed char)dp[16 * p_] << (8 * p_);
        }
        const long long x = (long long)(en >> 18);
        atomicAdd(rowesc + c, (unsigned long long)(x * (long long)(int)fw));
        atomicAdd(colesc + gi, (unsigned long long)(x * (long long)(int)fp));
      };
      const int ne = e_hi - e_lo;
      if (lane < ne) esc1(en0);
      if (64 + lane < ne) esc1(en1);
      for (int e = e_lo + 128 + lane; e < e_hi; e += 64) esc1(io.esc[e]);
    } else if (Y4) {
      const int64_t sc = (int64_t)st * 64;
      const int e1 = io.esc_off[kb + ((sc + 64 < RS) ? sc + 64 : RS)];
      const signed char* wd = reinterpret_cast<const signed char*>(Wr);
      for (int e = io.esc_off[kb + sc] + lane; e < e1; e += 64) {
        const unsigned en = io.esc[e];
        const int g = g0 + (int)((en >> 9) & 511u);
        const signed char* d = wd + ((int64_t)(g >> 6) * 64 + 16 * ((g >> 4) & 3)) * 16 + (g & 15);
        const long long x = (long long)d[0] + (long long)d[16] * 256ll + (long long)d[32] * 65536ll + (long long)d[48] * 16777216ll;
        atomicAdd(rowesc + ((en & 511u) & 63u), (unsigned long long)((long long)(en >> 18) * x));
      }
    }
    {
      const int t = j >> 2, p = j & 3;
#pragma unroll
      for (int r = 0; r < 4; ++r) {
        const int64_t n = cs + 16 * t + 4 * q + r;
        const int wb = p == 0 ? wtot[0] : p == 1 ? wtot[1] : p == 2 ? wtot[2] : wtot[3];
        const int ar = t == 0 ? acc_yw[0][r] : t == 1 ? acc_yw[1][r] : t == 2 ? acc_yw[2][r] : acc_yw[3][r];
        long long v = ((long long)ar + 128ll * (long long)wb) << (8 * p);
        if (Y4 && p == 0) v += (long long)rowesc[16 * t + 4 * q + r];
        v += __shfl_xor(v, 1, 64);
        v += __shfl_xor(v, 2, 64);
        if (p == 0 && n < N) io.YWpart[(int64_t)seg * N + n] = (float)ldexp((double)v, -e_w);
      }
      if (Y4) rowesc[lane] = 0ull;
    }
  }
  __syncthreads();
  int* comb = reinterpret_cast<int*>(ca_ys_lds);
#pragma unroll
  for (int a = 0; a < NP; ++a)
#pragma unroll
    for (int r = 0; r < 4; ++r) comb[((wv * NP + a) * 64 + lane) * 4 + r] = acc_yt[a][r];
  __syncthreads();
  if (Y4 && !OWN) {
    const signed char* pd = reinterpret_cast<const signed char*>(Pr);
    const int r = lane & 3;
    const int e1 = io.esc_off[kb + RS];
    for (int e = io.esc_off[kb] + (lane >> 2); e < e1; e += 16) {
      const unsigned en = io.esc[e];
      const int64_t n = c0 + (int64_t)(en & 511u);
      const int gi = (int)((en >> 9) & 511u);
      const int d = pd[((n >> 6) * 64 + 16 * ((n >> 4) & 3) + r) * 16 + (n & 15)];
      atomicAdd(comb + ((wv * NP + (gi >> 6)) * 64 + (gi & 63)) * 4 + r, (int)(en >> 18) * d);
    }
    __syncthreads();
  }
  long long pb[4] = {0, 0, 0, 0};
  if (!Y4) {
    const int64_t s0_ = ((int64_t)rg * 4 * RS) >> 6;
    const int64_t s1_ = (((int64_t)rg * 4 + 4) * RS < ((N + 63) / 64) * 64 ? ((int64_t)rg * 4 + 4) * RS : ((N + 63) / 64) * 64) >> 6;
    for (int64_t st = s0_; st < s1_; ++st) {
      const int4 d4 = *reinterpret_cast<const int4*>(io.Psum + st * 4);
      pb[0] += d4.x; pb[1] += d4.y; pb[2] += d4.z; pb[3] += d4.w;
    }
  }
  const double inv_p = ldexp(1.0, -io.exps[1]);
  for (int i = (int)threadIdx.x & (CA_YM_TB - 1); i < NP * 64; i += CA_YM_TB) {
    const int l = i & 63, a = i >> 6;
    double v = 0.0;
#pragma unroll
    for (int r = 3; r >= 0; --r) {
      const int o = i * 4 + r;
      const int sr = (comb[o] + comb[o + NP * 256]) + (comb[o + 2 * NP * 256] + comb[o + 3 * NP * 256]);
      v = v * 256.0 + (double)((long long)sr + 128 * pb[r]);
    }
    const int gl = 16 * (4 * a + (l >> 4)) + (l & 15), gene = g0 + gl;
    if (Y4L) v += (double)(long long)colesc[gl];
    io.YTpart[(int64_t)rg * Gp + gene] = (float)(v * inv_p);
  }
}
template <bool Y4>
__global__ void __launch_bounds__(CA_YM_TB, Y4 ? CA_YS4_WAVES : CA_YS_WAVES) k_ys_mfma(const uint8_t* __restrict__ Ys, ca_ys_io io, int64_t N, int Gp, int RS) {
  extern __shared__ __attribute__((aligned(16))) unsigned char ca_ys_dyn[];
  ca_ys_mfma_body<Y4 ? CA_YS4_DEPTH : CA_YS_DEPTH, Y4, true>((int)blockIdx.x, Ys, io, N, Gp, RS, ca_ys_dyn);
}
constexpr int CA_YS_LDS_BYTES = 4 * (CA_YS_GW / 64) * 64 * 4 * 4;
static_assert(4 * 64 * CA_YS_PITCH + 4 * 64 * 8 <= CA_YS_LDS_BYTES, "staging + row escapes fit the combine buffer");

struct ca_ysq_args {
  int nblk;
  const float* V; int Dv; int64_t G; int GS; const float* F; int Df; int64_t N; int64_t NS;
  const float* amax_in; int n_in; float slack_w, slack_p;
  float* amax_out;
  int* exps; uint4* Wr; uint4* Pr; int* Wsum; int* Psum;
};
__device__ __forceinline__ void ca_ys_quant_core(const ca_ysq_args& a, bool live, bool isw, int64_t step, const float (&vals)[16], float own,
                                                 int out, bool write_exps, float* sm ) {
  const int tid = threadIdx.x, l = tid & 63, wv = tid >> 6;
  float mw = 0.f, mp = 0.f;
  for (int i = tid; i < a.n_in; i += CA_YM_TB) { mw = fmaxf(mw, a.amax_in[2 * i]); mp = fmaxf(mp, a.amax_in[2 * i + 1]); }
#pragma unroll
  for (int o = 32; o > 0; o >>= 1) { mw = fmaxf(mw, __shfl_xor(mw, o, 64)); mp = fmaxf(mp, __shfl_xor(mp, o, 64)); }
  if (l == 0) { sm[2 * wv] = mw; sm[2 * wv + 1] = mp; }
  __syncthreads();
  mw = fmaxf(fmaxf(sm[0], sm[2]), fmaxf(sm[4], sm[6]));
  mp = fmaxf(fmaxf(sm[1], sm[3]), fmaxf(sm[5], sm[7]));
  __syncthreads();
  const int ew = ca_fix_exp(mw + a.slack_w), ep = ca_fix_exp(mp + a.slack_p);
  if (write_exps && tid == 0) { a.exps[0] = ew; a.exps[1] = ep; }
  float m = 0.f;
  if (live) {
    const float sc = ldexpf(1.f, isw ? ew : ep);
    const int p = l & 3;
    unsigned w[4] = {0u, 0u, 0u, 0u};
#pragma unroll
    for (int b = 0; b < 16; ++b) {
      const int x = (int)rintf(fminf(fmaxf(vals[b] * sc, -2147483000.f), 2147483000.f));
      w[b >> 2] |= ((unsigned)ca_digit(x, p) & 0xFFu) << (8 * (b & 3));
    }
    const uint4 v = {w[0], w[1], w[2], w[3]};
    (isw ? a.Wr : a.Pr)[step * 64 + l] = v;
    int sd = 0;
#pragma unroll
    for (int d = 0; d < 4; ++d)
#pragma unroll
      for (int b = 0; b < 4; ++b) sd += (int)(signed char)((w[d] >> (8 * b)) & 0xFFu);
    sd += __shfl_xor(sd, 16, 64);
    sd += __shfl_xor(sd, 32, 64);
    if (l < 4) (isw ? a.Wsum : a.Psum)[step * 4 + l] = sd;
    m = fabsf(own);
#pragma unroll
    for (int o = 32; o > 0; o >>= 1) m = fmaxf(m, __shfl_xor(m, o, 64));
  }
  if (l == 0) { sm[2 * wv] = isw ? m : 0.f; sm[2 * wv + 1] = isw ? 0.f : m; }
  __syncthreads();
  if (tid == 0) {
    a.amax_out[2 * out] = fmaxf(fmaxf(sm[0], sm[2]), fmaxf(sm[4], sm[6]));
    a.amax_out[2 * out + 1] = fmaxf(fmaxf(sm[1], sm[3]), fmaxf(sm[5], sm[7]));
  }
}
__device__ __forceinline__ void ca_ys_quant_body(int blk, const ca_ysq_args& a, float* sm ) {
  const int tid = threadIdx.x, l = tid & 63, wv = tid >> 6;
  const int64_t st = (int64_t)blk * (CA_YM_TB / 64) + wv;
  const bool live = st < a.GS + a.NS;
  const bool isw = !live || st < a.GS;
  const float* src = isw ? a.V : a.F;
  const int ld = isw ? a.Dv : a.Df;
  const int64_t rows = isw ? a.G : a.N, step = live ? (isw ? st : st - a.GS) : 0;
  float vals[16], own = 0.f;
  {
    const int64_t r0 = step * 64 + 16 * (l >> 4);
#pragma unroll
    for (int b = 0; b < 16; ++b) {
      const int64_t r = r0 + b;
      vals[b] = (live && r < rows) ? src[r * ld] : 0.f;
    }
    const int64_t r = step * 64 + l;
    if (live && r < rows) own = src[r * ld];
  }
  ca_ys_quant_core(a, live, isw, step, vals, own, blk, blk == 0, sm);
}
__device__ __forceinline__ float ca_ys_quant_wave(const ca_ysq_args& a, bool live, bool isw, int64_t step, float own, bool write_exps) {
  const int l = threadIdx.x & 63;
  float vals[16];
#pragma unroll
  for (int b = 0; b < 16; ++b) vals[b] = __shfl(own, 16 * (l >> 4) + b, 64);
  float mw = 0.f, mp = 0.f;
// ... 45 lines not shown
```

### clonealign_amd/csrc/clonealign_hip.hip

```cpp
#include "clonealign_hip.h"

#include <dlfcn.h>
#include <unistd.h>
#include <hip/hip_runtime.h>

#include <algorithm>
#include <cmath>
#include <cstdio>
#include <cstring>
#include <string>
#include <atomic>
#include <chrono>
#include <thread>
#include <vector>

#include "ca_kernels.hip.h"
#include "ca_poly.h"
#include "philox_host.h"

#include "ca_eng_state.inc"
#include "ca_eng_launch.inc"
#include "ca_eng_reduce.inc"
#include "ca_eng_loop.inc"
#include "ca_eng_ingest.inc"
// ... 107 lines not shown
  int ys_slot, ys_steps;
  int64_t look_slot;
  unsigned long long host_seq, host_seq_next;
  ca_small_args mon_tail;
  void take(const ca_engine* h) {
    gene_part = h->gene_part; gene_part_alt = h->gene_part_alt; gene_partB = h->gene_partB; gene_partB_alt = h->gene_partB_alt;
    pre_valid = h->pre_valid; em_stale = h->em_stale; yfin_pending = h->yfin_pending; ys_quant_ready = h->ys_quant_ready; ycache_valid = h->ycache_valid;
    look_valid = h->look_valid; bwd_ready = h->bwd_ready; ys_slot = h->ys_slot; ys_steps = h->ys_steps; look_slot = h->look_slot;
    host_seq = h->host_seq; host_seq_next = h->host_seq_next; mon_tail = h->mon_tail;
  }
  void restore(ca_engine* h) const {
    h->gene_part = gene_part; h->gene_part_alt = gene_part_alt; h->gene_partB = gene_partB; h->gene_partB_alt = gene_partB_alt;
    h->pre_valid = pre_valid; h->em_stale = em_stale; h->yfin_pending = yfin_pending; h->ys_quant_ready = ys_quant_ready; h->ycache_valid = ycache_valid;
    h->look_valid = look_valid; h->bwd_ready = bwd_ready; h->ys_slot = ys_slot; h->ys_steps = ys_steps; h->look_slot = look_slot;
    h->host_seq = host_seq; h->host_seq_next = host_seq_next; h->mon_tail = mon_tail;
  }
};
inline bool fwd_is_one_launch(const ca_engine* h, int64_t slotA, int64_t slotB) {
  return h->fused_ok && !h->s2 && h->fwd_cell && h->ride_ys && !h->ycache_valid && !h->y_defer && !h->y_pending && h->pre_valid && h->pre_A == slotA &&
         h->pre_B == slotB && h->ys_quant_ready && h->yfin_split && h->em_stale && h->D > 0 && h->tail_fuse && !is_sharded(h) && h->gate_local;
}
inline void gate_answer(ca_engine* h, int go) {
  volatile unsigned long long* w = reinterpret_cast<volatile unsigned long long*>(h->host_pinned + 48);
  std::atomic_thread_fence(std::memory_order_release);
  *w = (h->gate_seq << 1) | (unsigned long long)(go ? 1 : 0);
  std::atomic_thread_fence(std::memory_order_seq_cst);
}
int gate_resolve(ca_engine* h, int go) {
  gate_answer(h, go);
  if (!go) return 0;
  const double patience_us = (double)h->gate_ticks / h->ticks_per_us;
  const double us = std::chrono::duration<double, std::micro>(std::chrono::steady_clock::now() - h->gate_t0).count();
  if (patience_us >= 200.0 && us < 0.5 * patience_us) return 1;
  volatile unsigned long long* ack = reinterpret_cast<volatile unsigned long long*>(h->host_pinned + 56);
  unsigned spins = 0;
  auto t_next = std::chrono::steady_clock::now() + std::chrono::milliseconds(20);
  for (;;) {
    const unsigned long long a = *ack;
    if ((a >> 2) == h->gate_seq) return (a & 3ull) == 1ull ? 1 : 0;
    if ((++spins & 0x3FFu) == 0 && std::chrono::steady_clock::now() >= t_next) {
      t_next = std::chrono::steady_clock::now() + std::chrono::milliseconds(20);
      const hipError_t q = hipStreamQuery(h->stream);
      if (q == hipSuccess) {
        const unsigned long long a2 = *ack;
        if ((a2 >> 2) == h->gate_seq) return (a2 & 3ull) == 1ull ? 1 : 0;
        h->err = "ca_run: the gated update completed without leaving its verdict";
        return -CA_ERR_STATE;
      }
      if (q != hipErrorNotReady) { h->err = std::string("hipStreamQuery: ") + hipGetErrorString(q); return -CA_ERR_HIP; }
    }
  }
}
int gate_close(ca_engine* h) {
  if (!h->gate_open) return CA_OK;
  h->gate_open = false; h->gate_aborted = true;
  gate_answer(h, 0);
  HIPCK(h, hipStreamSynchronize(h->stream));
  if (h->gate_fsnap) h->gate_fsnap->restore(h);
  if (h->gate_snap) h->gate_snap->restore(h);
  return CA_OK;
}
#define CA_NOT_IN_RUN(h)                                                                                                                  \
  do {                                                                                                                                    \
    if ((h) && (h)->in_run) {                                                                                                             \
      (h)->err = "this call changes the engine's state and cannot be made from a ca_run_ex poll hook (read-only calls can: ca_get_param, " \
                 "ca_get_gradient, ca_get_info, ca_synchronize, ca_get_kernel_times)";                                                   \
      return CA_ERR_STATE;                                                                                                                \
    }                                                                                                                                     \
  } while (0)


static const char* sparse_descriptor_error(const ca_sparse* sp) {
  if (sp->kind != CA_SPARSE_CSR && sp->kind != CA_SPARSE_CSC) return "ca_sparse.kind must be CA_SPARSE_CSR or CA_SPARSE_CSC";
  if (sp->val_dtype < CA_F64 || sp->val_dtype > CA_U8) return "ca_sparse.val_dtype must be a ca_dtype";
  if (sp->index_bytes != 4 && sp->index_bytes != 8) return "ca_sparse.index_bytes must be 4 or 8";
  if (sp->nnz < 0) return "ca_sparse.nnz must not be negative";
  if (!sp->ptr || (sp->nnz > 0 && (!sp->idx || !sp->val))) return "ca_sparse: ptr, idx and val are required";
  return nullptr;
}

extern "C" {

int ca_abi_version(void) { return CA_ABI_VERSION; }
#ifdef CA_LAB
#include "../../tools/lab/ca_lab_host.inc"
#endif

int ca_device_count(int32_t* n) {
  int c = 0;
  const hipError_t e = hipGetDeviceCount(&c);
  if (e != hipSuccess) { (void)hipGetLastError(); c = 0; }
  if (n) *n = c;
  return e == hipSuccess ? CA_OK : CA_ERR_HIP;
}

int ca_default_options(ca_options* o) {
  if (!o) return CA_ERR_INVALID;
  memset(o, 0, sizeof(*o));
  o->learning_rate = 0.1;
  o->beta1 = 0.9; o->beta2 = 0.999; o->adam_eps = 1e-8;
  o->seed = 0x5eed5eedull;
  o->device = 0; o->y_storage = CA_YSTORE_AUTO; o->rank = 0; o->world = 1; o->profile = 0;
  return CA_OK;
}

const char* ca_last_error(ca_handle h) { return h ? h->err.c_str() : g_last_error.c_str(); }

static int create_common(const ca_problem* p, const ca_sparse* sp, const ca_options* o, ca_handle* out) {
  g_last_error.clear();
  if (!p || !out) { g_last_error = "null argument"; return CA_ERR_INVALID; }
  *out = nullptr;
  ca_options opt;
  if (o) opt = *o; else ca_default_options(&opt);
  auto bad = [&](const char* m) { g_last_error = m; return CA_ERR_INVALID; };
  if (p->N <= 0 || p->G <= 0 || p->C <= 0) return bad("N, G and C must be positive");
  if (p->C > 256) return bad("C > 256 clones not supported");
  if (p->K < 0 || p->P < 0 || p->S < 1) return bad("K >= 0, P >= 0, S >= 1 required");
  const int D = p->K > 0 ? p->K + p->P : 0;
  if (D > 8) return bad("K + P > 8 not supported");
  if (sp) {
    if (p->Y) return bad("ca_create_sparse: problem->Y must be NULL (the counts are the ca_sparse argument)");
    if (!p->L) return bad("L is required");
    const char* m = sparse_descriptor_error(sp);
    if (m) return bad(m);
  } else if (!p->Y || !p->L) return bad("Y and L are required");
  if (p->K > 0 && !p->psi0) return bad("psi0 is required when K > 0");
  if (p->P > 0 && !p->X) return bad("X is required when P > 0");
  if (opt.world < 1 || opt.rank < 0 || opt.rank >= opt.world) return bad("bad rank/world");
  if (opt.variant_on & CA_RETIRED_VARX)
    return bad("ca_options.variant_on asks for a variant that was removed (CA_VARX_Y_MFMA2, CA_VARX_RIDE_SEQ, CA_VARX_BAL_TILES: measured slower than what ships; "
               "the measurements are in DESIGN_HISTORY.md and profiles/, the code in the history)");
  if ((p->cell_index || p->gene_index) && (p->N_src < p->N || p->G_src < p->G)) return bad("N_src / G_src must be at least N / G when a selection is given");
  ca_engine* h = new ca_engine();
  h->N = p->N; h->G = p->G; h->C = p->C; h->K = p->K; h->P = p->P; h->S = p->S; h->D = D;
  h->layout = p->layout; h->opt = opt; h->device = opt.device;
  h->sp_in = sp;
  int rc;
  try { rc = create_impl(h, p); }
  catch (const std::exception& ex) { h->err = std::string("ca_create: ") + ex.what(); rc = CA_ERR_NOMEM; }
  if (rc != CA_OK) {
    g_last_error = h->err;
    ca_destroy(h);
    return rc;
  }
  h->sp_in = nullptr;
  *out = h;
  return CA_OK;
}

int ca_create(const ca_problem* p, const ca_options* o, ca_handle* out) { return create_common(p, nullptr, o, out); }

int ca_create_sparse(const ca_problem* p, const ca_sparse* y, const ca_options* o, ca_handle* out) {
  if (!y) { g_last_error = "null argument"; return CA_ERR_INVALID; }
  return create_common(p, y, o, out);
}

int ca_destroy(ca_handle h) {
  if (!h) return CA_OK;
  CA_NOT_IN_RUN(h);
  hipSetDevice(h->device);
  if (h->stream) hipStreamSynchronize(h->stream);
  if (h->stream2) { hipStreamSynchronize(h->stream2); hipStreamDestroy(h->stream2); }
  if (h->ev_params) hipEventDestroy(h->ev_params);
  if (h->ev_ydone) hipEventDestroy(h->ev_ydone);
  if (h->stream3) { hipStreamSynchronize(h->stream3); hipStreamDestroy(h->stream3); }
  if (h->ev_poly0) hipEventDestroy(h->ev_poly0);
  if (h->ev_poly1) hipEventDestroy(h->ev_poly1);
  if (h->ev_ywdone) hipEventDestroy(h->ev_ywdone);
  if (h->ev_stage) hipEventDestroy(h->ev_stage);
  if (h->comm) g_rccl.CommDestroy(h->comm);
  if (h->p2p) {
    for (void* q : h->p2p->opened) if (q) hipIpcCloseMemHandle(q);
    if (h->p2p->err_host) hipHostFree(h->p2p->err_host);
    if (h->p2p->err_local) hipFree(h->p2p->err_local);
    if (h->p2p->slab) hipFree(h->p2p->slab);
    if (h->p2p->peers_dev) hipFree(h->p2p->peers_dev);
    delete h->p2p;
  }
  for (auto& e : h->ev_pool) { hipEventDestroy(e.a); hipEventDestroy(e.b); }
  for (void* q : h->allocs) hipFree(q);
  if (h->eps_dev) hipFree(h->eps_dev);
  if (h->elbo_dev) hipFree(h->elbo_dev);
  if (h->host_pinned) hipHostFree(h->host_pinned);
  if (h->eps_stage) hipHostFree(h->eps_stage);
  if (h->host_ar_buf) hipHostFree(h->host_ar_buf);
  if (h->poly_ring) hipHostFree(h->poly_ring);
  if (h->stream) hipStreamDestroy(h->stream);
  delete h;
  return CA_OK;
}

int ca_get_info(ca_handle h, ca_info* i) {
  if (!h || !i) return CA_ERR_INVALID;
  memset(i, 0, sizeof(*i));
  i->N = h->N; i->G = h->G; i->C = h->C; i->K = h->K; i->P = h->P; i->S = h->S;
  i->y_storage = h->ystore; i->y_bytes_per_elem = h->ybytes; i->y_device_bytes = h->y_dev_bytes; i->device_bytes = h->dev_bytes;
  i->gsplit = h->gsplit; i->csplit = h->csplit; i->n_cu = h->n_cu; i->fused_sweep = h->fused_ok ? 1 : 0;
  i->fwd_mfma = ((h->fused_ok && h->fwd_mfma) || h->pfwd) ? 1 : 0; i->bwd_mfma = h->bwd_mfma ? 1 : 0; i->fsplit = h->fsplit; i->fwd_cell = (h->fused_ok && h->fwd_cell) ? 1 : 0;
  i->y_mfma = h->y_ys ? 2 : 0;
  i->y_stream_bits = h->y_ys ? (h->ys4 ? 4 : 8) : 0;
  i->y_ride = (h->ride_ok || h->ride_ys) ? 1 : 0;
  i->transport = (h->p2p && h->p2p->connected) ? CA_TRANSPORT_P2P : h->comm ? CA_TRANSPORT_RCCL : h->host_ar ? CA_TRANSPORT_HOST : CA_TRANSPORT_NONE;
  i->red_n = h->red_n;
  i->fwd_block_cells = (h->fused_ok && h->fwd_cell) ? 16 * h->fc_tl : 0; i->fwd_blocks_big = h->fc_nbig;
  i->fwd_balanced = h->fwd_bal ? h->bal_q : 0;
  i->fwd_series = h->poly ? 1 : 0; i->series_passes = h->n_series; i->series_fallbacks = h->n_series_fallback;
  i->mom_ride = h->mom_ride ? 1 : 0;
  i->cell_lean = h->cell_lean ? 1 : 0; i->cell_mfma = h->cell_mfma ? 1 : 0;
  i->mom_last = h->mom_last ? 1 : 0; i->mom_free_slots = h->mom_free_slots;
  i->fold_gsum = (h->fold_gsum && !is_sharded(h)) ? 1 : 0; i->yfin_split = (h->yfin_split && !is_sharded(h)) ? 1 : 0;
  i->update_merge = (h->upd_merge && h->fused_ok && h->fwd_cell && h->K > 0) ? 1 : 0;
  return CA_OK;
}

int ca_stream_busy(ca_handle h, int32_t* busy) {
  if (!h || !busy) return CA_ERR_INVALID;
  const hipError_t q = hipStreamQuery(h->stream);
  if (q != hipSuccess && q != hipErrorNotReady) HIPCK(h, q);
  *busy = q == hipErrorNotReady ? 1 : 0;
  if (q == hipErrorNotReady) (void)hipGetLastError();
  return CA_OK;
}

int ca_synchronize(ca_handle h) {
  if (!h) return CA_ERR_INVALID;
  HIPCK(h, hipSetDevice(h->device));
  CACK(gate_close(h));
  SYNC(h);
  return CA_OK;
}

#include "ca_eng_comm.inc"
static int stage_one(ca_handle h, const float* eps) { return stage_eps(h, eps, 1, 1); }

int ca_gamma_init(ca_handle h, const float* eps) {
  if (!h) return CA_ERR_INVALID;
  CA_NOT_IN_RUN(h);
  HIPCK(h, hipSetDevice(h->device));
  CACK(stage_one(h, eps));
  CACK(run_pass(h, 0, CA_MODE_GINIT, 0, nullptr));
  SYNC(h);
  return CA_OK;
}

int ca_elbo(ca_handle h, const float* eps, double* elbo) {
  if (!h || !elbo) return CA_ERR_INVALID;
  CA_NOT_IN_RUN(h);
  HIPCK(h, hipSetDevice(h->device));
  CACK(stage_one(h, eps));
  CACK(run_pass(h, 0, CA_MODE_ELBO, 0, h->elbo_dev));
  return read_doubles(h, h->elbo_dev, elbo, 1);
}

int ca_elbo_terms(ca_handle h, const float* eps, double terms[3]) {
  if (!h || !terms) return CA_ERR_INVALID;
  CA_NOT_IN_RUN(h);
  HIPCK(h, hipSetDevice(h->device));
  CACK(stage_one(h, eps));
  CACK(run_pass(h, 0, CA_MODE_ELBO, 0, h->elbo_dev));
  return read_doubles(h, h->terms_dev, terms, 3);
}

int ca_step(ca_handle h, const float* eps) {
  if (!h) return CA_ERR_INVALID;
  CA_NOT_IN_RUN(h);
  HIPCK(h, hipSetDevice(h->device));
  CACK(stage_one(h, eps));
  CACK(run_pass(h, 0, CA_MODE_TRAIN, 1, h->elbo_dev));
  SYNC(h);
  return CA_OK;
}

int ca_gradients(ca_handle h, const float* eps, double* elbo) {
  if (!h) return CA_ERR_INVALID;
  CA_NOT_IN_RUN(h);
  HIPCK(h, hipSetDevice(h->device));
  CACK(stage_one(h, eps));
  CACK(run_pass(h, 0, CA_MODE_TRAIN, 0, h->elbo_dev));
  double e;
  CACK(read_doubles(h, h->elbo_dev, &e, 1));
  if (elbo) *elbo = e;
  return CA_OK;
}
// ... 387 lines not shown
```

### clonealign_amd/engine.py

```python
import ctypes as C
import os

import numpy as np

_HERE = os.path.dirname(os.path.abspath(__file__))
LIB_PATH = os.path.join(_HERE, "libclonealign_hip.so")

CA_OK = 0
CA_ERR_NAN = 4
CA_INTERRUPTED = 7
CA_ABI_VERSION = 6
P2P_HANDLE_BYTES = 128
CA_F64, CA_F32, CA_I32, CA_U16, CA_U8 = 0, 1, 2, 3, 4
CA_ROW_MAJOR, CA_COL_MAJOR = 0, 1
YSTORE = {"auto": 0, "f32": 1, "u16": 2, "u8": 3}
YSTORE_NAME = {v: k for k, v in YSTORE.items()}
KERNEL_NAMES = ("fwd", "bwd", "ypass", "cell", "other")
VARIANTS = {"fused": 1 << 0, "fwd_mfma": 1 << 1, "fwd_cell": 1 << 2, "bwd_mfma": 1 << 3, "tail_fuse": 1 << 4, "async_y": 1 << 5,
            "pre": 1 << 6, "pair_elbo": 1 << 7, "prep_fast": 1 << 8, "update_merge": 1 << 9, "p2p": 1 << 10, "fold_gsum": 1 << 11, "y_ride": 1 << 12, "ride_seq": 1 << 13, "y_mfma1": 1 << 14, "yfin_ride": 1 << 15, "p2p_ride": 1 << 16, "run_gate": 1 << 17, "s2_fuse": 1 << 18, "fwd_bal": 1 << 19, "bwd_tl3": 1 << 20, "series": 1 << 21, "y4": 1 << 22, "mom_ride": 1 << 23, "cell_lean": 1 << 24, "mom_last": 1 << 25, "cell_mfma": 1 << 26}
VARIANTS_ON = {"y_mfma2": 1 << 0, "async_small": 1 << 1, "y_mfma1": 1 << 2, "fold_always": 1 << 3, "ride_seq": 1 << 4, "p2p_same_device": 1 << 5, "run_fwd": 1 << 6, "bal_tiles": 1 << 7, "series": 1 << 8, "y4": 1 << 9, "mom_last": 1 << 10}
OPT_VERBOSE = 0x80000000
TUNE = {"gsplit": 0, "fsplit": 1, "fc_tl": 2, "fc_nbig": 3, "csplit": 4, "csplit_m": 5, "tr": 6, "rg": 7}
TRANSPORT_NAME = {0: "none", 1: "rccl", 2: "host", 3: "p2p"}

EXPORTS = (
    "ca_abi_version", "ca_build_id", "ca_device_count", "ca_default_options", "ca_create", "ca_destroy", "ca_last_error", "ca_get_info",
    "ca_synchronize", "ca_stream_busy", "ca_comm_unique_id", "ca_comm_init", "ca_p2p_export", "ca_p2p_connect", "ca_p2p_commit", "ca_comm_benchmark", "ca_comm_selftest", "ca_set_host_allreduce", "ca_gamma_init", "ca_elbo", "ca_elbo_terms",
    "ca_step", "ca_gradients", "ca_run", "ca_run_ex", "ca_iterate", "ca_final_elbo", "ca_init_psi_pca", "ca_clone_gene_sums", "ca_get_param", "ca_set_param",
    "ca_get_gradient", "ca_reinit", "ca_get_kernel_times", "ca_reset_kernel_times", "ca_set_profile", "ca_eps_draw", "ca_allele_loglik", "ca_preprocess",
    "ca_group_create", "ca_group_destroy", "ca_group_last_error", "ca_group_get_info", "ca_group_rank_handle", "ca_group_init_psi_pca", "ca_group_gamma_init",
    "ca_group_elbo", "ca_group_step", "ca_group_run_ex", "ca_group_iterate", "ca_group_final_elbo", "ca_group_get_param", "ca_group_reinit",
    "ca_group_clone_gene_sums",
    "ca_create_sparse", "ca_group_create_sparse",
    "ca_fit_mse", "ca_group_fit_mse",
    "ca_logexpr_sums", "ca_group_logexpr_sums",
    "ca_clone_loglik", "ca_group_clone_loglik",
    "ca_project_cells", "ca_group_project_cells",
    "ca_clone_pair_loglik", "ca_group_clone_pair_loglik",
    "ca_clone_loglik_dm", "ca_group_clone_loglik_dm",
    "ca_clone_loglik_by_block", "ca_group_clone_loglik_by_block",
    "ca_simulate_counts", "ca_simulate_kernel_ms",
    "ca_predictive_stats", "ca_predictive_kernel_ms",
)
CA_SPARSE_CSR, CA_SPARSE_CSC = 0, 1


class CaProblem(C.Structure):
    _fields_ = [("N", C.c_int64), ("G", C.c_int32), ("C", C.c_int32), ("K", C.c_int32), ("P", C.c_int32),
                ("S", C.c_int32), ("layout", C.c_int32), ("y_dtype", C.c_int32), ("y_on_device", C.c_int32),
                ("Y", C.c_void_p), ("L", C.c_void_p), ("psi0", C.c_void_p), ("loc0", C.c_void_p),
                ("X", C.c_void_p), ("extra_loglik", C.c_void_p),
                ("N_src", C.c_int64), ("G_src", C.c_int32), ("cell_index", C.c_void_p), ("gene_index", C.c_void_p),
                ("y_ld", C.c_int64)]


class CaSparse(C.Structure):
    _fields_ = [("kind", C.c_int32), ("val_dtype", C.c_int32), ("index_bytes", C.c_int32), ("on_device", C.c_int32),
                ("nnz", C.c_int64), ("ptr", C.c_void_p), ("idx", C.c_void_p), ("val", C.c_void_p)]


class CaOptions(C.Structure):
    _fields_ = [("learning_rate", C.c_double), ("beta1", C.c_double), ("beta2", C.c_double),
                ("adam_eps", C.c_double), ("seed", C.c_uint64), ("device", C.c_int32),
                ("y_storage", C.c_int32), ("rank", C.c_int32), ("world", C.c_int32), ("profile", C.c_int32),
                ("variant_off", C.c_uint32), ("tune", C.c_int32 * 8), ("variant_on", C.c_uint32),
                ("ride_pattern", C.c_int32), ("comm_timeout_ms", C.c_int32), ("gate_timeout_us", C.c_int32), ("reserved", C.c_int32 * 2)]


class CaInfo(C.Structure):
    _fields_ = [("N", C.c_int64), ("G", C.c_int32), ("C", C.c_int32), ("K", C.c_int32), ("P", C.c_int32),
                ("S", C.c_int32), ("y_storage", C.c_int32), ("y_bytes_per_elem", C.c_int32),
                ("y_device_bytes", C.c_int64), ("device_bytes", C.c_int64), ("gsplit", C.c_int32),
                ("csplit", C.c_int32), ("n_cu", C.c_int32), ("fused_sweep", C.c_int32), ("fwd_mfma", C.c_int32),
                ("bwd_mfma", C.c_int32), ("fsplit", C.c_int32), ("fwd_cell", C.c_int32), ("y_mfma", C.c_int32),
                ("transport", C.c_int32), ("y_ride", C.c_int32), ("red_n", C.c_int64),
                ("fwd_block_cells", C.c_int32), ("fwd_blocks_big", C.c_int32), ("fold_gsum", C.c_int32), ("yfin_split", C.c_int32),
                ("update_merge", C.c_int32), ("fwd_balanced", C.c_int32), ("fwd_series", C.c_int32), ("y_stream_bits", C.c_int32),
                ("series_passes", C.c_int64), ("series_fallbacks", C.c_int64), ("mom_ride", C.c_int32), ("cell_lean", C.c_int32),
                ("mom_last", C.c_int32), ("mom_free_slots", C.c_int32), ("cell_mfma", C.c_int32)]


class CaGroupInfo(C.Structure):
    _fields_ = [("world", C.c_int32), ("transport", C.c_int32), ("p2p_status", C.c_int32), ("rccl_status", C.c_int32),
                ("rebuilds", C.c_int32), ("selftest_rounds", C.c_int32), ("N", C.c_int64), ("note", C.c_char * 384)]


class CaPreprocessParams(C.Structure):
    _fields_ = [("min_counts_per_gene", C.c_double), ("min_counts_per_cell", C.c_double),
                ("remove_outlying_genes", C.c_int32), ("remove_genes_same_copy_number", C.c_int32),
                ("nmads", C.c_double), ("max_copy_number", C.c_double)]


HOST_ALLREDUCE_FN = C.CFUNCTYPE(C.c_int, C.c_void_p, C.POINTER(C.c_double), C.c_int64)
POLL_FN = C.CFUNCTYPE(C.c_int, C.c_void_p, C.c_int32, C.c_double)

_lib = None


def load_library(path=None):
    global _lib
    if _lib is not None and path is None:
        return _lib
    p = path or os.environ.get("CLONEALIGN_HIP_LIB") or LIB_PATH
    if not os.path.exists(p):
        raise RuntimeError(
            f"{p} not found: build the HIP engine first (python -c 'import __graft_entry__ as g; g.build()' "
            "or make -C clonealign_amd/csrc). clonealign_amd has no CPU fallback.")
    lib = C.CDLL(p)
    lib.ca_last_error.restype = C.c_char_p
    lib.ca_last_error.argtypes = [C.c_void_p]
    lib.ca_build_id.restype = C.c_char_p
    lib.ca_build_id.argtypes = []
    lib.ca_group_last_error.restype = C.c_char_p
    lib.ca_group_last_error.argtypes = [C.c_void_p]
    for name in EXPORTS:
        if name not in ("ca_last_error", "ca_build_id", "ca_group_last_error"):
            getattr(lib, name).restype = C.c_int
    lib.ca_device_count.argtypes = [C.POINTER(C.c_int32)]
    lib.ca_create.argtypes = [C.POINTER(CaProblem), C.POINTER(CaOptions), C.POINTER(C.c_void_p)]
    lib.ca_create_sparse.argtypes = [C.POINTER(CaProblem), C.POINTER(CaSparse), C.POINTER(CaOptions), C.POINTER(C.c_void_p)]
    lib.ca_destroy.argtypes = [C.c_void_p]
    lib.ca_get_info.argtypes = [C.c_void_p, C.POINTER(CaInfo)]
    lib.ca_synchronize.argtypes = [C.c_void_p]
    lib.ca_stream_busy.argtypes = [C.c_void_p, C.POINTER(C.c_int32)]
    lib.ca_comm_unique_id.argtypes = [C.c_char_p]
    lib.ca_comm_init.argtypes = [C.c_void_p, C.c_char_p]
    lib.ca_p2p_export.argtypes = [C.c_void_p, C.c_char_p]
    lib.ca_p2p_connect.argtypes = [C.c_void_p, C.c_char_p]
    lib.ca_p2p_commit.argtypes = [C.c_void_p, C.c_int32]
    lib.ca_comm_benchmark.argtypes = [C.c_void_p, C.c_int32, C.c_int32, C.c_int64, C.POINTER(C.c_double)]
    lib.ca_comm_selftest.argtypes = [C.c_void_p, C.c_int32, C.c_int64, C.POINTER(C.c_int64)]
    lib.ca_set_host_allreduce.argtypes = [C.c_void_p, HOST_ALLREDUCE_FN, C.c_void_p]
    lib.ca_gamma_init.argtypes = [C.c_void_p, C.c_void_p]
    lib.ca_elbo.argtypes = [C.c_void_p, C.c_void_p, C.POINTER(C.c_double)]
    lib.ca_elbo_terms.argtypes = [C.c_void_p, C.c_void_p, C.POINTER(C.c_double)]
    lib.ca_step.argtypes = [C.c_void_p, C.c_void_p]
    lib.ca_gradients.argtypes = [C.c_void_p, C.c_void_p, C.POINTER(C.c_double)]
    lib.ca_run.argtypes = [C.c_void_p, C.c_int32, C.c_double, C.c_void_p, C.c_int64, C.c_void_p,
                           C.POINTER(C.c_int32)]
    lib.ca_run_ex.argtypes = [C.c_void_p, C.c_int32, C.c_double, C.c_void_p, C.c_int64, C.c_void_p,
                              C.POINTER(C.c_int32), POLL_FN, C.c_void_p]
    lib.ca_iterate.argtypes = [C.c_void_p, C.c_int32, C.c_void_p, C.c_int64, C.POINTER(C.c_double)]
    lib.ca_final_elbo.argtypes = [C.c_void_p, C.c_int32, C.c_void_p, C.c_int64, C.c_void_p,
                                  C.POINTER(C.c_double), C.POINTER(C.c_double)]
    lib.ca_init_psi_pca.argtypes = [C.c_void_p, C.c_void_p, C.c_int32, C.c_uint64, C.c_void_p]
    lib.ca_clone_gene_sums.argtypes = [C.c_void_p, C.c_void_p, C.c_void_p, C.c_void_p]
    lib.ca_fit_mse.argtypes = [C.c_void_p, C.c_void_p, C.c_void_p, C.POINTER(C.c_double), C.POINTER(C.c_int64), C.c_void_p, C.c_void_p]
    lib.ca_logexpr_sums.argtypes = [C.c_void_p, C.c_void_p, C.c_int32, C.c_void_p, C.c_void_p, C.c_void_p, C.c_void_p]
    lib.ca_clone_loglik.argtypes = [C.c_void_p, C.c_void_p, C.c_void_p, C.c_void_p, C.c_int32, C.c_int32, C.c_void_p]
    lib.ca_clone_pair_loglik.argtypes = [C.c_void_p, C.c_void_p, C.c_void_p, C.c_void_p, C.c_int32, C.c_int32, C.c_void_p, C.c_int32, C.c_int64, C.c_int64,
                                         C.c_void_p, C.c_void_p]
    lib.ca_clone_loglik_dm.argtypes = lib.ca_clone_pair_loglik.argtypes
    lib.ca_clone_loglik_by_block.argtypes = [C.c_void_p, C.c_void_p, C.c_void_p, C.c_void_p, C.c_int32, C.c_int32, C.c_void_p, C.c_int32, C.c_int64, C.c_int64,
                                             C.c_void_p, C.c_void_p, C.c_void_p, C.c_void_p]
    lib.ca_project_cells.argtypes = [C.c_void_p, C.c_void_p, C.c_void_p, C.c_int32, C.c_int32, C.c_void_p, C.c_void_p, C.c_void_p, C.c_int32, C.c_int32,
                                     C.c_double, C.c_double, C.c_void_p, C.c_void_p, C.c_void_p, C.c_void_p, C.c_void_p, C.c_void_p]
    lib.ca_simulate_counts.argtypes = [C.c_int64, C.c_int32, C.c_int32, C.c_int32, C.c_void_p, C.c_void_p, C.c_void_p, C.c_void_p, C.c_void_p, C.c_uint64, C.c_uint64,
                                       C.c_int64, C.c_int32, C.c_void_p, C.c_char_p]
    lib.ca_simulate_kernel_ms.argtypes = [C.POINTER(C.c_double)]
    lib.ca_predictive_stats.argtypes = [C.c_int64, C.c_int32, C.c_int32, C.c_int32, C.c_void_p, C.c_void_p, C.c_void_p, C.c_void_p, C.c_void_p, C.c_uint64, C.c_uint64,
                                        C.c_int32, C.c_int64, C.c_int32, C.c_void_p, C.c_void_p, C.c_char_p]
    lib.ca_predictive_kernel_ms.argtypes = [C.POINTER(C.c_double)]
# ... 881 lines not shown
```

### include/clonealign_hip.h

```cpp
#ifndef CLONEALIGN_HIP_H
#define CLONEALIGN_HIP_H

#include <stdint.h>

#ifdef __cplusplus
extern "C" {
#endif

#define CA_ABI_VERSION 6

typedef struct ca_engine* ca_handle;

enum ca_status {
  CA_OK = 0,
  CA_ERR_INVALID = 1,
  CA_ERR_HIP = 2,
  CA_ERR_NOMEM = 3,
  CA_ERR_NAN = 4,
  CA_ERR_COMM = 5,
  CA_ERR_STATE = 6,
  CA_INTERRUPTED = 7
};

enum ca_dtype { CA_F64 = 0, CA_F32 = 1, CA_I32 = 2, CA_U16 = 3, CA_U8 = 4 };
enum ca_layout { CA_ROW_MAJOR = 0, CA_COL_MAJOR = 1 };
enum ca_ystore { CA_YSTORE_AUTO = 0, CA_YSTORE_F32 = 1, CA_YSTORE_U16 = 2, CA_YSTORE_U8 = 3 };

typedef struct ca_problem {
  int64_t N;
  int32_t G, C;
  int32_t K, P, S;
  int32_t layout;
  int32_t y_dtype;
  int32_t y_on_device;
  const void* Y;
  const double* L;
  const double* psi0;
  const double* loc0;
  const double* X;
  const double* extra_loglik;
  int64_t N_src;
  int32_t G_src;
  const int64_t* cell_index;
  const int32_t* gene_index;
  int64_t y_ld;
} ca_problem;

enum ca_variant {
  CA_VAR_FUSED = 1 << 0,
  CA_VAR_FWD_MFMA = 1 << 1,
  CA_VAR_FWD_CELL = 1 << 2,
  CA_VAR_BWD_MFMA = 1 << 3,
  CA_VAR_TAIL_FUSE = 1 << 4,
  CA_VAR_ASYNC_Y = 1 << 5,
  CA_VAR_PRE = 1 << 6,
  CA_VAR_PAIR_ELBO = 1 << 7,
  CA_VAR_PREP_FAST = 1 << 8,
  CA_VAR_UPDATE_MERGE = 1 << 9,
  CA_VAR_P2P_RIDE = 1 << 16,
  CA_VAR_RUN_GATE = 1 << 17,
  CA_VAR_S2_FUSE = 1 << 18,
  CA_VAR_FWD_BAL = 1 << 19,
  CA_VAR_BWD_TL3 = 1 << 20,
  CA_VAR_SERIES = 1 << 21,
  CA_VAR_P2P = 1 << 10,
  CA_VAR_FOLD_GSUM = 1 << 11,
  CA_VAR_Y_RIDE = 1 << 12,
  CA_VAR_Y_MFMA1 = 1 << 14,
  CA_VAR_YFIN_RIDE = 1 << 15,
  CA_VAR_Y4 = 1 << 22,
  CA_VAR_MOM_RIDE = 1 << 23,
  CA_VAR_CELL_LEAN = 1 << 24,
  CA_VAR_MOM_LAST = 1 << 25,
  CA_VAR_CELL_MFMA = 1 << 26,
  CA_VAR_RIDE_SEQ = 1 << 13
};
enum ca_variant_on {
  CA_VARX_Y_MFMA2 = 1 << 0,
  CA_VARX_Y_MFMA1 = 1 << 2,
  CA_VARX_FOLD_ALWAYS = 1 << 3,
  CA_VARX_RIDE_SEQ = 1 << 4,
  CA_VARX_P2P_SAME_DEVICE = 1 << 5,
  CA_VARX_RUN_FWD = 1 << 6,
  CA_VARX_BAL_TILES = 1 << 7,
  CA_VARX_SERIES = 1 << 8,
  CA_VARX_Y4 = 1 << 9,
  CA_VARX_MOM_LAST = 1 << 10,
  CA_VARX_ASYNC_SMALL = 1 << 1
};
#define CA_OPT_VERBOSE 0x80000000u
enum ca_tune_id {
  CA_TUNE_GSPLIT = 0, CA_TUNE_FSPLIT = 1, CA_TUNE_FC_TL = 2, CA_TUNE_FC_NBIG = 3, CA_TUNE_CSPLIT = 4, CA_TUNE_CSPLIT_M = 5,
  CA_TUNE_TR = 6, CA_TUNE_RG = 7, CA_TUNE_COUNT = 8
};

typedef struct ca_options {
  double learning_rate;
  double beta1, beta2, adam_eps;
  uint64_t seed;
  int32_t device;
  int32_t y_storage;
  int32_t rank, world;
  int32_t profile;
  uint32_t variant_off;
  int32_t tune[8];
  uint32_t variant_on;
  int32_t ride_pattern;
  int32_t comm_timeout_ms;
  int32_t gate_timeout_us;
  int32_t reserved[2];
} ca_options;

typedef struct ca_info {
  int64_t N;
  int32_t G, C, K, P, S;
  int32_t y_storage;
  int32_t y_bytes_per_elem;
  int64_t y_device_bytes;
  int64_t device_bytes;
  int32_t gsplit, csplit;
  int32_t n_cu;
  int32_t fused_sweep;
  int32_t fwd_mfma;
  int32_t bwd_mfma;
  int32_t fsplit;
  int32_t fwd_cell;
  int32_t y_mfma;
  int32_t transport;
  int32_t y_ride;
  int64_t red_n;
  int32_t fwd_block_cells;
  int32_t fwd_blocks_big;
  int32_t fold_gsum;
  int32_t yfin_split;
  int32_t update_merge;
  int32_t fwd_balanced;
  int32_t fwd_series;
  int32_t y_stream_bits;
  int64_t series_passes;
  int64_t series_fallbacks;
  int32_t mom_ride;
  int32_t cell_lean;
  int32_t mom_last;
  int32_t mom_free_slots;
  int32_t cell_mfma;
} ca_info;
enum ca_transport { CA_TRANSPORT_NONE = 0, CA_TRANSPORT_RCCL = 1, CA_TRANSPORT_HOST = 2, CA_TRANSPORT_P2P = 3 };

enum ca_kernel_id {
  CA_KERNEL_FWD = 0,
  CA_KERNEL_BWD = 1,
  CA_KERNEL_YPASS = 2,
  CA_KERNEL_CELL = 3,
  CA_KERNEL_OTHER = 4,
  CA_KERNEL_COUNT = 5
};

int ca_abi_version(void);
const char* ca_build_id(void);
int ca_device_count(int32_t* n);
int ca_default_options(ca_options* opts);

int ca_create(const ca_problem* problem, const ca_options* opts, ca_handle* out);

enum ca_sparse_kind { CA_SPARSE_CSR = 0,
                      CA_SPARSE_CSC = 1 };
typedef struct ca_sparse {
  int32_t kind;
  int32_t val_dtype;
  int32_t index_bytes;
  int32_t on_device;
  int64_t nnz;
  const void* ptr;
  const void* idx;
  const void* val;
} ca_sparse;
int ca_create_sparse(const ca_problem* problem, const ca_sparse* y, const ca_options* opts, ca_handle* out);
int ca_destroy(ca_handle h);
const char* ca_last_error(ca_handle h);
int ca_get_info(ca_handle h, ca_info* info);
int ca_synchronize(ca_handle h);
int ca_stream_busy(ca_handle h, int32_t* busy);

int ca_comm_unique_id(char id[128]);
int ca_comm_init(ca_handle h, const char id[128]);
#define CA_P2P_HANDLE_BYTES 128
int ca_p2p_export(ca_handle h, char handle[CA_P2P_HANDLE_BYTES]);
int ca_p2p_connect(ca_handle h, const char* handles );
int ca_p2p_commit(ca_handle h, int32_t all_ranks_ok);
int ca_comm_benchmark(ca_handle h, int32_t transport, int32_t n_calls, int64_t n_doubles, double* us_per_call);
int ca_comm_selftest(ca_handle h, int32_t n_rounds, int64_t n_doubles, int64_t* n_bad);
typedef int (*ca_host_allreduce_fn)(void* user, double* buf, int64_t n);
int ca_set_host_allreduce(ca_handle h, ca_host_allreduce_fn fn, void* user);

int ca_gamma_init(ca_handle h, const float* eps);
int ca_elbo(ca_handle h, const float* eps, double* elbo);
int ca_elbo_terms(ca_handle h, const float* eps, double terms[3]);
int ca_step(ca_handle h, const float* eps);
int ca_gradients(ca_handle h, const float* eps, double* elbo);

int ca_run(ca_handle h, int32_t max_iter, double rel_tol, const float* eps_stream, int64_t n_draws,
           double* elbo_trace, int32_t* n_elbo);
typedef int (*ca_poll_fn)(void* user, int32_t iter, double elbo);
int ca_run_ex(ca_handle h, int32_t max_iter, double rel_tol, const float* eps_stream, int64_t n_draws,
              double* elbo_trace, int32_t* n_elbo, ca_poll_fn poll, void* user);
int ca_iterate(ca_handle h, int32_t n_iter, const float* eps_stream, int64_t n_draws, double* last_elbo);
int ca_final_elbo(ca_handle h, int32_t n_rep, const float* eps_stream, int64_t n_draws, double* values,
                  double* mean, double* sd);

int ca_init_psi_pca(ca_handle h, const double* noise, int32_t n_iter, uint64_t seed, double* pcs_out);

int ca_clone_gene_sums(ca_handle h, const int32_t* clone_of_cell, double* T, double* Syy);

int ca_fit_mse(ca_handle h, const int32_t* clone_of_cell, const double* E, double* sse_total, int64_t* n_cells_used,
               double* sse_gene, double* sse_cell);

int ca_clone_loglik(ca_handle h, const double* E , const double* U , const double* V ,
                    int32_t D, int32_t with_const, double* ll );

int ca_clone_pair_loglik(ca_handle h, const double* E , const double* U , const double* V , int32_t D,
                         int32_t with_const, const double* weights , int32_t n_weights, int64_t cell_lo, int64_t cell_cnt,
                         double* ll , double* pair_ll );

int ca_clone_loglik_dm(ca_handle h, const double* E , const double* U , const double* V , int32_t D,
                       int32_t with_const, const double* conc , int32_t n_conc, int64_t cell_lo, int64_t cell_cnt,
                       double* ll , double* dm_ll );

int ca_clone_loglik_by_block(ca_handle h, const double* E , const double* U , const double* V , int32_t D,
// ... 105 lines not shown
```

Baseline: 9275 iterations/s.

## Add mixed 2-bit/4-bit count image with per-segment gene permutation

Adds a compressed Y image for the int8 MFMA count pass. Within each 512-gene segment, genes are sorted by how often they hold counts of 3 or more. The sparsest 64-gene groups are stored as 2-bit values and the rest as 4-bit, with larger values going to an escape list. The aim is to cut the bytes the Y streaming kernel reads each iteration. In exchange it adds setup work (histogram, host planning, a second escape table), permutation gathers and LDS reshuffles in the kernel, and more escape handling.

```diff
diff --git a/clonealign_amd/csrc/ca_eng_create.inc b/clonealign_amd/csrc/ca_eng_create.inc
--- a/clonealign_amd/csrc/ca_eng_create.inc
+++ b/clonealign_amd/csrc/ca_eng_create.inc
@@ -25,6 +25,35 @@
   const int per = ca_mom_last_per(a);
   if (per < 1 || per > CA_ML_MAX_PER) return false;
   return CA_ML_STREAM_FIXED_US + (double)a.image_bytes / CA_ML_STREAM_BYTES_PER_US >= CA_ML_MIN_STREAM_US;
+}
+
+constexpr int CA_Y2_NS[2] = {6, 5};
+constexpr double CA_Y2_MIN_COUNTS = 2.0e8;
+inline int ca_y2_plan_impl(const int32_t* cnt3, const int32_t* cnt15, int Gp, int64_t counts, int force_n2, uint16_t* perm, uint16_t* pos, int64_t* n_esc) {
+  const int nseg = Gp / CA_YS_GW;
+  int64_t e15 = 0, e3[CA_YS_GW / 64 + 1];
+  for (int b = 0; b <= CA_YS_GW / 64; ++b) e3[b] = 0;
+  std::vector<int> idx(CA_YS_GW);
+  for (int s = 0; s < nseg; ++s) {
+    const int32_t* c3 = cnt3 + (size_t)s * CA_YS_GW;
+    const int32_t* c15 = cnt15 + (size_t)s * CA_YS_GW;
+    for (int i = 0; i < CA_YS_GW; ++i) idx[i] = i;
+    std::stable_sort(idx.begin(), idx.end(), [&](int a, int b) { return c3[a] < c3[b]; });
+    for (int i = 0; i < CA_YS_GW; ++i) {
+      perm[(size_t)s * CA_YS_GW + i] = (uint16_t)idx[i];
+      pos[(size_t)s * CA_YS_GW + idx[i]] = (uint16_t)i;
+      e15 += c15[idx[i]];
+      e3[i / 64 + 1] += (int64_t)c3[idx[i]] - c15[idx[i]];
+    }
+  }
+  for (int b = 1; b <= CA_YS_GW / 64; ++b) e3[b] += e3[b - 1];
+  int n2 = 0;
+  if (force_n2 > 0) n2 = force_n2 < CA_YS_GW / 64 ? force_n2 : CA_YS_GW / 64 - 1;
+  else
+    for (int k = 0; k < 2 && n2 == 0; ++k)
+      if ((e15 + e3[CA_Y2_NS[k]]) * 256 <= counts) n2 = CA_Y2_NS[k];
+  *n_esc = e15 + e3[n2];
+  return n2;
 }
 
 int create_impl(ca_engine* h, const ca_problem* p) {
@@ -336,7 +365,7 @@
     h->ys_RS = 64;
     while (h->ys_RS < 512 && cdiv(Nn, 4 * h->ys_RS) * h->ys_nseg > 4 * h->n_cu) h->ys_RS *= 2;
     h->ys_nrg = cdiv(Nn, 4 * h->ys_RS);
-    const bool y4_force = variantx_on(h, CA_VARX_Y4, "CA_Y4_ON");
+    const bool y4_force = variantx_on(h, CA_VARX_Y4, "CA_Y4_ON") || variantx_on(h, CA_VARX_Y2, "CA_Y2_ON");
     if (variant_on(h, CA_VAR_Y4, "CA_Y4") && (h->poly || y4_force) && (double)Nn * (double)h->Gp < 2.0e9) {
       const int64_t nkeys = (int64_t)h->ys_nrg * h->ys_nseg * 4 * h->ys_RS;
       CACK(dalloc(h, &h->esc_off, nkeys + 1));
@@ -383,6 +412,50 @@
       hipLaunchKernelGGL(k_bias_y, dim3(cdiv(h->ys_N64 * (h->Gp / 16), CA_YM_TB)), dim3(CA_YM_TB), 0, h->stream, (const uint8_t*)h->Y, (uint4*)h->Ys, Nn,
                          h->ys_N64, h->Gp);
     HIPCK(h, hipGetLastError());
+    if (h->ys4 && h->poly && variant_on(h, CA_VAR_Y2, "CA_Y2")) {
+      const bool y2_force = variantx_on(h, CA_VARX_Y2, "CA_Y2_ON");
+      const int lab_n2 = (h->opt.reserved[0] >> 8) & 15;
+      if (y2_force || (double)h->ys_N64 * (double)h->Gp >= CA_Y2_MIN_COUNTS) {
+        int* hist = nullptr;
+        CACK(dalloc(h, &hist, 2 * (int64_t)h->Gp));
+        hipLaunchKernelGGL(k_y2_hist, dim3(cdiv(h->Gp / 4, CA_YM_TB), (unsigned)cdiv(Nn, 64)), dim3(CA_YM_TB), 0, h->stream, (const uint8_t*)h->Y, Nn, h->Gp, hist);
+        HIPCK(h, hipGetLastError());
+        std::vector<int32_t> hc(2 * (size_t)h->Gp);
+        HIPCK(h, hipMemcpyAsync(hc.data(), hist, hc.size() * sizeof(int32_t), hipMemcpyDeviceToHost, h->stream));
+        SYNC(h);
+        std::vector<uint16_t> perm(h->Gp), pos(h->Gp);
+        int64_t ne = 0;
+        const int n2 = ca_y2_plan_impl(hc.data(), hc.data() + h->Gp, h->Gp, Nn * (int64_t)h->G, y2_force ? (lab_n2 == 5 || lab_n2 == 6 ? lab_n2 : 6) : 0, perm.data(), pos.data(), &ne);
+        if (n2 > 0 && ne < ((int64_t)1 << 31)) {
+          CACK(dalloc(h, &h->y2_perm, (int64_t)h->Gp));
+          CACK(dalloc(h, &h->y2_pos, (int64_t)h->Gp));
+          HIPCK(h, hipMemcpyAsync(h->y2_perm, perm.data(), (size_t)h->Gp * 2, hipMemcpyHostToDevice, h->stream));
+          HIPCK(h, hipMemcpyAsync(h->y2_pos, pos.data(), (size_t)h->Gp * 2, hipMemcpyHostToDevice, h->stream));
+          const int64_t nkeys = (int64_t)h->ys_nrg * h->ys_nseg * 4 * h->ys_RS, nw = Nn * h->ys_nseg;
+          CACK(dalloc(h, &h->esc2_off, nkeys + 1));
+          hipLaunchKernelGGL(k_esc_count, dim3(cdiv(nw * 64, CA_YM_TB)), dim3(CA_YM_TB), 0, h->stream, (const uint8_t*)h->Y, Nn, h->Gp, h->ys_nseg, h->ys_RS,
+                             h->esc2_off, (const uint4*)h->y2_pos, n2);
+          hipLaunchKernelGGL(k_esc_scan, dim3(1), dim3(1024), 0, h->stream, h->esc2_off, nkeys);
+          HIPCK(h, hipGetLastError());
+          int total = 0;
+          HIPCK(h, hipMemcpyAsync(&total, h->esc2_off + nkeys, sizeof(int), hipMemcpyDeviceToHost, h->stream));
+          SYNC(h);
+          if ((int64_t)total != ne) { h->err = "2-bit image: the device's escape count differs from the host plan's"; return CA_ERR_STATE; }
+          h->n_esc2 = total;
+          CACK(dalloc(h, &h->esc2, h->n_esc2));
+          hipLaunchKernelGGL(k_esc_fill, dim3(cdiv(nw * 64, CA_YM_TB)), dim3(CA_YM_TB), 0, h->stream, (const uint8_t*)h->Y, Nn, h->Gp, h->ys_nseg, h->ys_RS,
+                             h->esc2_off, h->esc2, (const uint4*)h->y2_pos, n2);
+          const int64_t sb = n2 * 1024 + (8 - n2) * 2048, ib = (h->ys_N64 / 64) * h->ys_nseg * sb;
+          CACK(dalloc(h, &h->Ys2, ib));
+          hipLaunchKernelGGL(k_pack_y2, dim3(cdiv(ib / 16, CA_YM_TB)), dim3(CA_YM_TB), 0, h->stream, (const uint8_t*)h->Y, (uint4*)h->Ys2, Nn, h->ys_N64, h->Gp, n2,
+                             h->y2_perm);
+          HIPCK(h, hipGetLastError());
+          SYNC(h);
+          h->ys_n2 = n2;
+          h->y_dev_bytes += ib + 4 * h->n_esc2 + 4 * (nkeys + 1) + 4 * (int64_t)h->Gp;
+        }
+      }
+    }
     if (h->adam_bound > 0) h->ys_step_bound = (float)(1.02 * h->adam_bound);
     h->y_ys = true;
     h->y_dev_bytes += h->ys4 ? h->ys_N64 * h->Gp / 2 + 4 * h->n_esc + 4 * ((int64_t)h->ys_nrg * h->ys_nseg * 4 * h->ys_RS + 1) : h->ys_N64 * h->Gp;
diff --git a/clonealign_amd/csrc/ca_eng_loop.inc b/clonealign_amd/csrc/ca_eng_loop.inc
--- a/clonealign_amd/csrc/ca_eng_loop.inc
+++ b/clonealign_amd/csrc/ca_eng_loop.inc
@@ -102,6 +102,7 @@
   io.Wr = h->Wr; io.Pr = h->Pr; io.Wsum = h->Wsum; io.Psum = h->Psum; io.exps = h->ys_exps + 2 * h->ys_slot;
   io.YWpart = h->YWpart; io.YTpart = h->YTpart;
   io.esc_off = h->ys4 ? h->esc_off : nullptr; io.esc = h->ys4 ? h->esc : nullptr;
+  io.perm = nullptr;
   return io;
 }
 ca_ovf_args ys_ovf(ca_engine* h) { return ovf_args(h, h->YWpart + (int64_t)h->ys_nseg * h->N); }
@@ -119,9 +120,12 @@
   h->ycache_valid = true;
   return CA_OK;
 }
-template <bool Y4>
+template <bool Y4, int N2 = 0>
 void launch_ys(ca_engine* h) {
   constexpr int lds = Y4 ? CA_YS4_LDS_BYTES : CA_YS_LDS_BYTES;
+  ca_ys_io yio = ys_io(h);
+  const uint8_t* Yimg = h->Ys;
+  if (N2 > 0) { Yimg = h->Ys2; yio.esc_off = h->esc2_off; yio.esc = h->esc2; yio.perm = h->y2_perm; }
   const int nb_main = h->ys_nrg * h->ys_nseg;
   const ca_pm_args* pm = h->mom_args;
   h->mom_args = nullptr;
@@ -132,17 +136,19 @@
     if (pm) {
       ca_pm_args pmo = *pm;
       if (h->mom_last && h->mom_ovf_first) pmo.blk0 += ovf.nb_rows + ovf.nb_chunks;
-      hipLaunchKernelGGL(k_ys_mfma_ovf_mom<Y4>, grid, dim3(CA_YM_TB), lds, h->stream, h->Ys, ys_io(h), h->N, h->Gp, h->ys_RS, nb_main, ovf, h->F, h->V, h->D, pmo);
-    }
-    else hipLaunchKernelGGL(k_ys_mfma_ovf<Y4>, grid, dim3(CA_YM_TB), lds, h->stream, h->Ys, ys_io(h), h->N, h->Gp, h->ys_RS, nb_main, ovf, h->F, h->V, h->D);
+      hipLaunchKernelGGL((k_ys_mfma_ovf_mom<Y4, N2>), grid, dim3(CA_YM_TB), lds, h->stream, Yimg, yio, h->N, h->Gp, h->ys_RS, nb_main, ovf, h->F, h->V, h->D, pmo);
+    }
+    else hipLaunchKernelGGL((k_ys_mfma_ovf<Y4, N2>), grid, dim3(CA_YM_TB), lds, h->stream, Yimg, yio, h->N, h->Gp, h->ys_RS, nb_main, ovf, h->F, h->V, h->D);
   } else {
-    if (pm) hipLaunchKernelGGL(k_ys_mfma_mom<Y4>, dim3(nmom + nb_main), dim3(CA_YM_TB), lds, h->stream, h->Ys, ys_io(h), h->N, h->Gp, h->ys_RS, *pm);
-    else hipLaunchKernelGGL(k_ys_mfma<Y4>, dim3(nb_main), dim3(CA_YM_TB), lds, h->stream, h->Ys, ys_io(h), h->N, h->Gp, h->ys_RS);
+    if (pm) hipLaunchKernelGGL((k_ys_mfma_mom<Y4, N2>), dim3(nmom + nb_main), dim3(CA_YM_TB), lds, h->stream, Yimg, yio, h->N, h->Gp, h->ys_RS, *pm);
+    else hipLaunchKernelGGL((k_ys_mfma<Y4, N2>), dim3(nb_main), dim3(CA_YM_TB), lds, h->stream, Yimg, yio, h->N, h->Gp, h->ys_RS);
   }
 }
 int ycache_ys(ca_engine* h) {
   CACK(ys_quant(h));
-  if (h->ys4) LAUNCH(h, CA_KERNEL_YPASS, launch_ys<true>(h));
+  if (h->ys4 && h->ys_n2 == 6) LAUNCH(h, CA_KERNEL_YPASS, (launch_ys<true, 6>(h)));
+  else if (h->ys4 && h->ys_n2 == 5) LAUNCH(h, CA_KERNEL_YPASS, (launch_ys<true, 5>(h)));
+  else if (h->ys4) LAUNCH(h, CA_KERNEL_YPASS, launch_ys<true>(h));
   else LAUNCH(h, CA_KERNEL_YPASS, launch_ys<false>(h));
   const bool defer = h->ys_defer_next;
   h->ys_defer_next = false;
diff --git a/clonealign_amd/csrc/ca_eng_state.inc b/clonealign_amd/csrc/ca_eng_state.inc
--- a/clonealign_amd/csrc/ca_eng_state.inc
+++ b/clonealign_amd/csrc/ca_eng_state.inc
@@ -170,6 +170,7 @@
   uint64_t draw = 0;
   hipEvent_t ev_ywdone = nullptr; bool yw_pending = false, on_side = false;
   bool y_ys = false, ys4 = false; int* esc_off = nullptr; unsigned* esc = nullptr; int64_t n_esc = 0;
+  int ys_n2 = 0; uint8_t* Ys2 = nullptr; unsigned short *y2_perm = nullptr, *y2_pos = nullptr; int* esc2_off = nullptr; unsigned* esc2 = nullptr; int64_t n_esc2 = 0;
   uint8_t* Ys = nullptr; uint4 *Wr = nullptr, *Pr = nullptr; int *Wsum = nullptr, *Psum = nullptr;
   int* ys_exps = nullptr;
   unsigned* ys_amax = nullptr;
diff --git a/clonealign_amd/csrc/ca_kernels.hip.h b/clonealign_amd/csrc/ca_kernels.hip.h
--- a/clonealign_amd/csrc/ca_kernels.hip.h
+++ b/clonealign_amd/csrc/ca_kernels.hip.h
@@ -700,7 +700,7 @@
   }
 }
 
-template <bool Y4>
+template <bool Y4, int N2 = 0>
 __global__ void __launch_bounds__(CA_YM_TB, Y4 ? CA_YS4_WAVES : CA_YS_WAVES) k_ys_mfma_ovf(const uint8_t* __restrict__ Ys, ca_ys_io io, int64_t N, int Gp, int RS,
                                                                        int nb_main, ca_ovf_args ovf, const float* __restrict__ F,
                                                                        const float* __restrict__ V, int Dstride) {
@@ -711,19 +711,19 @@
     return;
   }
   extern __shared__ __attribute__((aligned(16))) unsigned char ca_ys_dyn[];
-  ca_ys_mfma_body<Y4 ? CA_YS4_DEPTH : CA_YS_DEPTH, Y4, true>((int)blockIdx.x, Ys, io, N, Gp, RS, ca_ys_dyn);
+  ca_ys_mfma_body<Y4 ? CA_YS4_DEPTH : CA_YS_DEPTH, Y4, true, N2>((int)blockIdx.x, Ys, io, N, Gp, RS, ca_ys_dyn);
 }
 
 #include "ca_polymom.hip.h"
 static_assert(sizeof(ca_pm_lds) <= (size_t)CA_YS_LDS_BYTES && sizeof(ca_pm_lds) <= (size_t)CA_YS4_LDS_BYTES, "the moment role's tables fit the stream's dynamic LDS");
-template <bool Y4>
+template <bool Y4, int N2 = 0>
 __global__ void __launch_bounds__(CA_YM_TB, Y4 ? CA_YS4_WAVES : CA_YS_WAVES) k_ys_mfma_mom(const uint8_t* __restrict__ Ys, ca_ys_io io, int64_t N, int Gp, int RS, ca_pm_args pm) {
   extern __shared__ __attribute__((aligned(16))) unsigned char ca_ys_dyn[];
   const int nmom = pm.nmb + pm.nred, rb = (int)blockIdx.x - pm.blk0;
   if (rb >= 0 && rb < nmom) { ca_pm_ride_block<CA_YM_TB>(pm, rb, ca_ys_dyn); return; }
-  ca_ys_mfma_body<Y4 ? CA_YS4_DEPTH : CA_YS_DEPTH, Y4, true>(rb < 0 ? (int)blockIdx.x : (int)blockIdx.x - nmom, Ys, io, N, Gp, RS, ca_ys_dyn);
-}
-template <bool Y4>
+  ca_ys_mfma_body<Y4 ? CA_YS4_DEPTH : CA_YS_DEPTH, Y4, true, N2>(rb < 0 ? (int)blockIdx.x : (int)blockIdx.x - nmom, Ys, io, N, Gp, RS, ca_ys_dyn);
+}
+template <bool Y4, int N2 = 0>
 __global__ void __launch_bounds__(CA_YM_TB, Y4 ? CA_YS4_WAVES : CA_YS_WAVES) k_ys_mfma_ovf_mom(const uint8_t* __restrict__ Ys, ca_ys_io io, int64_t N, int Gp, int RS,
                                                                            int nb_main, ca_ovf_args ovf, const float* __restrict__ F,
                                                                            const float* __restrict__ V, int Dstride, ca_pm_args pm) {
@@ -737,7 +737,7 @@
     else ca_ovf_chunks_body(b - ovf.nb_rows, ovf.chunk_start, ovf.row2, ovf.val2, F, Dstride, ovf.csum, ovf.nchunk, 1, 0);
     return;
   }
-  ca_ys_mfma_body<Y4 ? CA_YS4_DEPTH : CA_YS_DEPTH, Y4, true>(blk, Ys, io, N, Gp, RS, ca_ys_dyn);
+  ca_ys_mfma_body<Y4 ? CA_YS4_DEPTH : CA_YS_DEPTH, Y4, true, N2>(blk, Ys, io, N, Gp, RS, ca_ys_dyn);
 }
 
 struct ca_ysride_args {
diff --git a/clonealign_amd/csrc/ca_ymfma.hip.h b/clonealign_amd/csrc/ca_ymfma.hip.h
--- a/clonealign_amd/csrc/ca_ymfma.hip.h
+++ b/clonealign_amd/csrc/ca_ymfma.hip.h
@@ -77,13 +77,25 @@
   for (int b = 0; b < 4; ++b) c += (((v.x >> (8 * b)) & 0xFFu) >= 15u) + (((v.y >> (8 * b)) & 0xFFu) >= 15u);
   return c;
 }
-__global__ void __launch_bounds__(CA_YM_TB) k_esc_count(const uint8_t* __restrict__ Y, int64_t N, int Gp, int nseg, int RS, int* __restrict__ off) {
+__device__ __forceinline__ unsigned ca_esc_pos(const uint4& p8, int b) { return ((b < 2 ? p8.x : b < 4 ? p8.y : b < 6 ? p8.z : p8.w) >> (16 * (b & 1))) & 0xFFFFu; }
+__device__ __forceinline__ int ca_esc_count8_y2(uint2 v, uint4 p8, int n2) {
+  int c = 0;
+#pragma unroll
+  for (int b = 0; b < 8; ++b) {
+    const unsigned y = ((b < 4 ? v.x : v.y) >> (8 * (b & 3))) & 0xFFu;
+    c += y >= ((int)ca_esc_pos(p8, b) < 64 * n2 ? 3u : 15u);
+  }
+  return c;
+}
+__global__ void __launch_bounds__(CA_YM_TB) k_esc_count(const uint8_t* __restrict__ Y, int64_t N, int Gp, int nseg, int RS, int* __restrict__ off,
+                                                        const uint4* __restrict__ pos8 = nullptr, int n2 = 0) {
   const int64_t w = ((int64_t)blockIdx.x * CA_YM_TB + threadIdx.x) >> 6;
   const int lane = threadIdx.x & 63;
   if (w >= N * nseg) return;
   const int64_t n = w / nseg;
   const int seg = (int)(w - n * nseg);
-  int c = ca_esc_count8(*reinterpret_cast<const uint2*>(Y + n * (int64_t)Gp + seg * 512 + 8 * lane));
+  const uint2 v = *reinterpret_cast<const uint2*>(Y + n * (int64_t)Gp + seg * 512 + 8 * lane);
+  int c = pos8 ? ca_esc_count8_y2(v, pos8[seg * 64 + lane], n2) : ca_esc_count8(v);
 #pragma unroll
   for (int o = 32; o > 0; o >>= 1) c += __shfl_xor(c, o, 64);
   if (lane == 0) off[ca_esc_key(n, seg, nseg, RS)] = c;
@@ -107,14 +119,16 @@
   if (t == 1023) off[n] = (int)sm[1023];
 }
 __global__ void __launch_bounds__(CA_YM_TB) k_esc_fill(const uint8_t* __restrict__ Y, int64_t N, int Gp, int nseg, int RS, const int* __restrict__ off,
-                                                       unsigned* __restrict__ esc) {
+                                                       unsigned* __restrict__ esc, const uint4* __restrict__ pos8 = nullptr, int n2 = 0) {
   const int64_t w = ((int64_t)blockIdx.x * CA_YM_TB + threadIdx.x) >> 6;
   const int lane = threadIdx.x & 63;
   if (w >= N * nseg) return;
   const int64_t n = w / nseg;
   const int seg = (int)(w - n * nseg);
   const uint2 v = *reinterpret_cast<const uint2*>(Y + n * (int64_t)Gp + seg * 512 + 8 * lane);
-  const int c = ca_esc_count8(v);
+  uint4 p8 = {0u, 0u, 0u, 0u};
+  if (pos8) p8 = pos8[seg * 64 + lane];
+  const int c = pos8 ? ca_esc_count8_y2(v, p8, n2) : ca_esc_count8(v);
   int x = c;
 #pragma unroll
   for (int o = 1; o < 64; o <<= 1) { const int u = __shfl_up(x, o, 64); if (lane >= o) x += u; }
@@ -123,8 +137,68 @@
 #pragma unroll
   for (int b = 0; b < 8; ++b) {
     const unsigned y = ((b < 4 ? v.x : v.y) >> (8 * (b & 3))) & 0xFFu;
-    if (y >= 15u) esc[e++] = cl | ((unsigned)(8 * lane + b) << 9) | ((y - 15u) << 18);
-  }
+    const unsigned pos = pos8 ? ca_esc_pos(p8, b) : (unsigned)(8 * lane + b);
+    const unsigned thr = (pos8 && (int)pos < 64 * n2) ? 3u : 15u;
+    if (y >= thr) esc[e++] = cl | (pos << 9) | ((y - thr) << 18);
+  }
+}
+__global__ void __launch_bounds__(CA_YM_TB) k_y2_hist(const uint8_t* __restrict__ Y, int64_t N, int Gp, int* __restrict__ hist) {
+  const int g = 4 * ((int)blockIdx.x * CA_YM_TB + threadIdx.x);
+  if (g >= Gp) return;
+  const int64_t n0 = (int64_t)blockIdx.y * 64, n1 = n0 + 64 < N ? n0 + 64 : N;
+  unsigned c3 = 0u, c15 = 0u;
+  for (int64_t n = n0; n < n1; ++n) {
+    const unsigned v = *reinterpret_cast<const unsigned*>(Y + n * (int64_t)Gp + g);
+#pragma unroll
+    for (int b = 0; b < 4; ++b) {
+      const unsigned y = (v >> (8 * b)) & 0xFFu;
+      c3 += (unsigned)(y >= 3u) << (8 * b);
+      c15 += (unsigned)(y >= 15u) << (8 * b);
+    }
+  }
+#pragma unroll
+  for (int b = 0; b < 4; ++b) {
+    const int a3 = (int)((c3 >> (8 * b)) & 0xFFu), a15 = (int)((c15 >> (8 * b)) & 0xFFu);
+    if (a3) atomicAdd(hist + g + b, a3);
+    if (a15) atomicAdd(hist + Gp + g + b, a15);
+  }
+}
+__global__ void __launch_bounds__(CA_YM_TB) k_pack_y2(const uint8_t* __restrict__ Y, uint4* __restrict__ Y2, int64_t N, int64_t N64, int Gp, int n2,
+                                                      const unsigned short* __restrict__ perm) {
+  const int64_t i = (int64_t)blockIdx.x * CA_YM_TB + threadIdx.x;
+  const int nseg = Gp / 512, sb = n2 * 64 + (8 - n2) * 128;
+  if (i >= (N64 / 64) * nseg * sb) return;
+  const int64_t unit = i / sb, cs = unit / nseg;
+  const int seg = (int)(unit - cs * nseg), r = (int)(i - unit * sb);
+  const bool nar = r < n2 * 64;
+  const int rw = r - n2 * 64;
+  const int a = nar ? r >> 6 : n2 + (rw >> 7), l = nar ? r & 63 : rw & 63, ld = nar ? 0 : (rw >> 6) & 1;
+  const int j = l & 15, q = l >> 4;
+  const unsigned short* pp = perm + seg * 512 + 64 * a + 16 * q;
+  const uint8_t* base = Y + seg * 512;
+  unsigned w[4] = {0u, 0u, 0u, 0u};
+#pragma unroll
+  for (int gb = 0; gb < 16; ++gb) {
+    const uint8_t* col = base + pp[gb];
+    unsigned x = 0u;
+    if (nar) {
+#pragma unroll
+      for (int t = 0; t < 4; ++t) {
+        const int64_t n = cs * 64 + 16 * t + j;
+        const unsigned y = n < N ? col[n * (int64_t)Gp] : 0u;
+        x |= (y < 3u ? y : 3u) << (2 * t);
+      }
+    } else {
+#pragma unroll
+      for (int t = 0; t < 2; ++t) {
+        const int64_t n = cs * 64 + 32 * ld + 16 * t + j;
+        const unsigned y = n < N ? col[n * (int64_t)Gp] : 0u;
+        x |= (y < 15u ? y : 15u) << (4 * t);
+      }
+    }
+    w[gb >> 2] |= x << (8 * (gb & 3));
+  }
+  Y2[i] = (uint4){w[0], w[1], w[2], w[3]};
 }
 
 __device__ __forceinline__ ca_i32x4 ca_mfma_i8(uint4 a, uint4 b, ca_i32x4 c) {
@@ -168,6 +242,7 @@
   const uint4* Wr; const uint4* Pr; const int* Wsum; const int* Psum; const int* exps;
   float* YWpart; float* YTpart;
   const int* esc_off; const unsigned* esc;
+  const unsigned short* perm;
 };
 #ifndef CA_YS4_DEPTH
 #define CA_YS4_DEPTH 4
@@ -182,7 +257,7 @@
 constexpr int CA_YS4_LDS_BYTES = CA_YS4_OFF_COL + CA_YS_GW * 8;
 static_assert(CA_YS4_OFF_PSI + 4 * 256 <= CA_YS4_OFF_COL, "the 4-bit launch's tables fit below its column-escape sums");
 static_assert(4 * CA_YS4_LDS_BYTES <= 160 * 1024, "four blocks of the 4-bit launch per CU");
-template <int DEPTH = CA_YS_DEPTH, bool Y4 = false, bool OWN = false>
+template <int DEPTH = CA_YS_DEPTH, bool Y4 = false, bool OWN = false, int N2 = 0>
 __device__ __forceinline__ void ca_ys_mfma_body(int blk, const uint8_t* __restrict__ Ys, const ca_ys_io& io, int64_t N, int Gp,
                                                 int RS ,
                                                 unsigned char* ca_ys_lds ) {
@@ -191,6 +266,8 @@
   constexpr bool Y4L = Y4 && OWN;
   constexpr int NP = CA_YS_GW / 64;
   static_assert(NP % DEPTH == 0, "pieces per cell step must be a multiple of the pipeline depth");
+  static_assert(N2 == 0 || (Y4 && OWN && N2 < NP), "the 2-bit blocks belong to the 4-bit image's own launch");
+  constexpr int SB2 = N2 * 1024 + (NP - N2) * 2048;
   const int lane = threadIdx.x & 63, j = lane & 15, q = lane >> 4;
   const int wv = __builtin_amdgcn_readfirstlane((int)(threadIdx.x >> 6) & 3);
   const int nseg = Gp / CA_YS_GW;
@@ -211,7 +288,8 @@
   const unsigned char* rd_row = my + j * CA_YS_PITCH + 16 * q;
   const unsigned rd_tr = (unsigned)(size_t)my + (unsigned)((16 * q + (j >> 1)) * CA_YS_PITCH + 8 * (j & 1));
   constexpr int PB = Y4 ? 2048 : 4096, NL = PB / 1024;
-  const uint8_t* src = Ys + ((c0 >> 6) * (int64_t)(Gp / 64) + (g0 >> 6)) * PB;
+  const uint8_t* src = N2 > 0 ? Ys + ((c0 >> 6) * (int64_t)nseg + seg) * SB2
+                              : Ys + ((c0 >> 6) * (int64_t)(Gp / 64) + (g0 >> 6)) * PB;
   const uint4* wsrc = Wr + (int64_t)(g0 >> 6) * 64;
   const unsigned voff = 16u * (unsigned)lane;
   uint4 R[DEPTH][NL], W[DEPTH];
@@ -221,9 +299,10 @@
   const __amdgpu_buffer_rsrc_t rw = __builtin_amdgcn_make_buffer_rsrc(const_cast<uint4*>(wsrc), 0, NP * 1024, 0x00020000);
   const __amdgpu_buffer_rsrc_t rp = __builtin_amdgcn_make_buffer_rsrc(const_cast<uint4*>(Pr + (c0 >> 6) * 64), 0, 0x7FFFFFFF, 0x00020000);
   auto issue = [&](int slot, int st, int a, unsigned vo) {
-    const int so = (st * (Gp / 64) + a) * PB;
+    const int so = N2 > 0 ? st * nseg * SB2 + (a < N2 ? a * 1024 : N2 * 1024 + (a - N2) * 2048) : (st * (Gp / 64) + a) * PB;
 #pragma unroll
     for (int i = 0; i < NL; ++i) {
+      if (N2 > 0 && i > 0 && a < N2) continue;
       const ca_v4u v = __builtin_amdgcn_raw_buffer_load_b128(ry, (int)(vo + 1024u * (unsigned)i), so, 2 );
       R[slot][i] = (uint4){v.x, v.y, v.z, v.w};
     }
@@ -234,11 +313,18 @@
   };
   uint4* wl = reinterpret_cast<uint4*>(ca_ys_lds + CA_YS4_OFF_W);
   unsigned long long* colesc = reinterpret_cast<unsigned long long*>(ca_ys_lds + CA_YS4_OFF_COL);
-  uint4 wimg[2];
+  uint4 wimg[2], pidx[2][2];
   int eoff = 0;
   if (Y4L) {
     wimg[0] = wsrc[threadIdx.x];
     wimg[1] = wsrc[threadIdx.x + CA_YM_TB];
+    if (N2 > 0) {
+#pragma unroll
+      for (int h2 = 0; h2 < 2; ++h2) {
+        const uint4* pq = reinterpret_cast<const uint4*>(io.perm + g0 + 16 * (((int)threadIdx.x + h2 * CA_YM_TB) >> 4));
+        pidx[h2][0] = pq[0]; pidx[h2][1] = pq[1];
+      }
+    }
     if (lane <= nsteps) eoff = io.esc_off[((int64_t)blk * 4 + wv) * RS + (64 * lane < RS ? 64 * lane : RS)];
   }
   uint4 pr_nx = {0u, 0u, 0u, 0u};
@@ -252,6 +338,25 @@
   }
   if (Y4L) {
     static_assert(2 * CA_YM_TB == CA_YS_GW, "the block's threads hold the segment's W image and column sums in two halves");
+    if (N2 > 0) {
+      uint4* tmp = reinterpret_cast<uint4*>(ca_ys_lds);
+      tmp[threadIdx.x] = wimg[0];
+      tmp[threadIdx.x + CA_YM_TB] = wimg[1];
+      __syncthreads();
+      const unsigned char* tb = reinterpret_cast<const unsigned char*>(tmp) + 16 * ((int)threadIdx.x & 3);
+#pragma unroll
+      for (int h2 = 0; h2 < 2; ++h2) {
+        unsigned w4[4] = {0u, 0u, 0u, 0u};
+#pragma unroll
+        for (int b = 0; b < 16; ++b) {
+          const uint4& pv = pidx[h2][b >> 3];
+          const unsigned two = (b & 7) < 2 ? pv.x : (b & 7) < 4 ? pv.y : (b & 7) < 6 ? pv.z : pv.w;
+          const int gi = (int)((two >> (16 * (b & 1))) & 511u);
+          w4[b >> 2] |= (unsigned)tb[((gi >> 6) * 64 + 16 * ((gi >> 4) & 3)) * 16 + (gi & 15)] << (8 * (b & 3));
+        }
+        wimg[h2] = (uint4){w4[0], w4[1], w4[2], w4[3]};
+      }
+    }
     wl[threadIdx.x] = wimg[0];
     wl[threadIdx.x + CA_YM_TB] = wimg[1];
     colesc[threadIdx.x] = 0ull;
@@ -305,9 +410,10 @@
       if (Y4) {
 #pragma unroll
         for (int t = 0; t < 4; ++t) {
-          const uint4 v = R[slot][t >> 1];
-          const int sh = 4 * (t & 1);
-          const uint4 av = ca_and4((uint4){v.x >> sh, v.y >> sh, v.z >> sh, v.w >> sh}, 0x0F0F0F0Fu);
+          const bool nar = N2 > 0 && a < N2;
+          const uint4 v = R[slot][nar ? 0 : t >> 1];
+          const int sh = nar ? 2 * t : 4 * (t & 1);
+          const uint4 av = ca_and4((uint4){v.x >> sh, v.y >> sh, v.z >> sh, v.w >> sh}, nar ? 0x03030303u : 0x0F0F0F0Fu);
           *reinterpret_cast<uint4*>(const_cast<unsigned char*>(rd_row) + 16 * t * CA_YS_PITCH) = av;
           acc_yw[t] = ca_mfma_i8(av, wr, acc_yw[t]);
         }
@@ -437,15 +543,15 @@
       const int sr = (comb[o] + comb[o + NP * 256]) + (comb[o + 2 * NP * 256] + comb[o + 3 * NP * 256]);
       v = v * 256.0 + (double)((long long)sr + 128 * pb[r]);
     }
-    const int gl = 16 * (4 * a + (l >> 4)) + (l & 15), gene = g0 + gl;
+    const int gl = 16 * (4 * a + (l >> 4)) + (l & 15), gene = g0 + (N2 > 0 ? (int)io.perm[g0 + gl] : gl);
     if (Y4L) v += (double)(long long)colesc[gl];
     io.YTpart[(int64_t)rg * Gp + gene] = (float)(v * inv_p);
   }
 }
-template <bool Y4>
+template <bool Y4, int N2 = 0>
 __global__ void __launch_bounds__(CA_YM_TB, Y4 ? CA_YS4_WAVES : CA_YS_WAVES) k_ys_mfma(const uint8_t* __restrict__ Ys, ca_ys_io io, int64_t N, int Gp, int RS) {
   extern __shared__ __attribute__((aligned(16))) unsigned char ca_ys_dyn[];
-  ca_ys_mfma_body<Y4 ? CA_YS4_DEPTH : CA_YS_DEPTH, Y4, true>((int)blockIdx.x, Ys, io, N, Gp, RS, ca_ys_dyn);
+  ca_ys_mfma_body<Y4 ? CA_YS4_DEPTH : CA_YS_DEPTH, Y4, true, N2>((int)blockIdx.x, Ys, io, N, Gp, RS, ca_ys_dyn);
 }
 constexpr int CA_YS_LDS_BYTES = 4 * (CA_YS_GW / 64) * 64 * 4 * 4;
 static_assert(4 * 64 * CA_YS_PITCH + 4 * 64 * 8 <= CA_YS_LDS_BYTES, "staging + row escapes fit the combine buffer");
diff --git a/clonealign_amd/csrc/clonealign_hip.hip b/clonealign_amd/csrc/clonealign_hip.hip
--- a/clonealign_amd/csrc/clonealign_hip.hip
+++ b/clonealign_amd/csrc/clonealign_hip.hip
@@ -213,6 +213,10 @@
 extern "C" {
 
 int ca_abi_version(void) { return CA_ABI_VERSION; }
+int ca_y2_plan(const int32_t* cnt3, const int32_t* cnt15, int32_t Gp, int64_t counts, int32_t force_n2, uint16_t* perm, uint16_t* pos, int64_t* n_esc) {
+  if (!cnt3 || !cnt15 || !perm || !pos || !n_esc || Gp <= 0 || Gp % CA_YS_GW != 0 || force_n2 < 0) return CA_ERR_INVALID;
+  return ca_y2_plan_impl(cnt3, cnt15, Gp, counts, force_n2, perm, pos, n_esc);
+}
 #ifdef CA_LAB
 #include "../../tools/lab/ca_lab_host.inc"
 #endif
@@ -330,6 +334,10 @@
   i->fwd_mfma = ((h->fused_ok && h->fwd_mfma) || h->pfwd) ? 1 : 0; i->bwd_mfma = h->bwd_mfma ? 1 : 0; i->fsplit = h->fsplit; i->fwd_cell = (h->fused_ok && h->fwd_cell) ? 1 : 0;
   i->y_mfma = h->y_ys ? 2 : 0;
   i->y_stream_bits = h->y_ys ? (h->ys4 ? 4 : 8) : 0;
+  i->y_stream_n2 = h->ys_n2;
+  i->y_stream_esc = h->ys_n2 > 0 ? h->n_esc2 : h->ys4 ? h->n_esc : 0;
+  i->y_stream_bytes = !h->y_ys ? 0 : h->ys_n2 > 0 ? (h->ys_N64 / 64) * (int64_t)h->ys_nseg * (h->ys_n2 * 1024 + (8 - h->ys_n2) * 2048) + 4 * h->n_esc2
+                                   : h->ys4 ? h->ys_N64 * h->Gp / 2 + 4 * h->n_esc : h->ys_N64 * h->Gp;
   i->y_ride = (h->ride_ok || h->ride_ys) ? 1 : 0;
   i->transport = (h->p2p && h->p2p->connected) ? CA_TRANSPORT_P2P : h->comm ? CA_TRANSPORT_RCCL : h->host_ar ? CA_TRANSPORT_HOST : CA_TRANSPORT_NONE;
   i->red_n = h->red_n;
diff --git a/clonealign_amd/engine.py b/clonealign_amd/engine.py
--- a/clonealign_amd/engine.py
+++ b/clonealign_amd/engine.py
@@ -17,8 +17,8 @@
 YSTORE_NAME = {v: k for k, v in YSTORE.items()}
 KERNEL_NAMES = ("fwd", "bwd", "ypass", "cell", "other")
 VARIANTS = {"fused": 1 << 0, "fwd_mfma": 1 << 1, "fwd_cell": 1 << 2, "bwd_mfma": 1 << 3, "tail_fuse": 1 << 4, "async_y": 1 << 5,
-            "pre": 1 << 6, "pair_elbo": 1 << 7, "prep_fast": 1 << 8, "update_merge": 1 << 9, "p2p": 1 << 10, "fold_gsum": 1 << 11, "y_ride": 1 << 12, "ride_seq": 1 << 13, "y_mfma1": 1 << 14, "yfin_ride": 1 << 15, "p2p_ride": 1 << 16, "run_gate": 1 << 17, "s2_fuse": 1 << 18, "fwd_bal": 1 << 19, "bwd_tl3": 1 << 20, "series": 1 << 21, "y4": 1 << 22, "mom_ride": 1 << 23, "cell_lean": 1 << 24, "mom_last": 1 << 25, "cell_mfma": 1 << 26}
-VARIANTS_ON = {"y_mfma2": 1 << 0, "async_small": 1 << 1, "y_mfma1": 1 << 2, "fold_always": 1 << 3, "ride_seq": 1 << 4, "p2p_same_device": 1 << 5, "run_fwd": 1 << 6, "bal_tiles": 1 << 7, "series": 1 << 8, "y4": 1 << 9, "mom_last": 1 << 10}
+            "pre": 1 << 6, "pair_elbo": 1 << 7, "prep_fast": 1 << 8, "update_merge": 1 << 9, "p2p": 1 << 10, "fold_gsum": 1 << 11, "y_ride": 1 << 12, "ride_seq": 1 << 13, "y_mfma1": 1 << 14, "yfin_ride": 1 << 15, "p2p_ride": 1 << 16, "run_gate": 1 << 17, "s2_fuse": 1 << 18, "fwd_bal": 1 << 19, "bwd_tl3": 1 << 20, "series": 1 << 21, "y4": 1 << 22, "mom_ride": 1 << 23, "cell_lean": 1 << 24, "mom_last": 1 << 25, "cell_mfma": 1 << 26, "y2": 1 << 27}
+VARIANTS_ON = {"y_mfma2": 1 << 0, "async_small": 1 << 1, "y_mfma1": 1 << 2, "fold_always": 1 << 3, "ride_seq": 1 << 4, "p2p_same_device": 1 << 5, "run_fwd": 1 << 6, "bal_tiles": 1 << 7, "series": 1 << 8, "y4": 1 << 9, "mom_last": 1 << 10, "y2": 1 << 11}
 OPT_VERBOSE = 0x80000000
 TUNE = {"gsplit": 0, "fsplit": 1, "fc_tl": 2, "fc_nbig": 3, "csplit": 4, "csplit_m": 5, "tr": 6, "rg": 7}
 TRANSPORT_NAME = {0: "none", 1: "rccl", 2: "host", 3: "p2p"}
@@ -77,7 +77,8 @@
                 ("fwd_block_cells", C.c_int32), ("fwd_blocks_big", C.c_int32), ("fold_gsum", C.c_int32), ("yfin_split", C.c_int32),
                 ("update_merge", C.c_int32), ("fwd_balanced", C.c_int32), ("fwd_series", C.c_int32), ("y_stream_bits", C.c_int32),
                 ("series_passes", C.c_int64), ("series_fallbacks", C.c_int64), ("mom_ride", C.c_int32), ("cell_lean", C.c_int32),
-                ("mom_last", C.c_int32), ("mom_free_slots", C.c_int32), ("cell_mfma", C.c_int32)]
+                ("mom_last", C.c_int32), ("mom_free_slots", C.c_int32), ("cell_mfma", C.c_int32),
+                ("y_stream_n2", C.c_int32), ("y_stream_esc", C.c_int64), ("y_stream_bytes", C.c_int64)]
 
 
 class CaGroupInfo(C.Structure):
diff --git a/include/clonealign_hip.h b/include/clonealign_hip.h
--- a/include/clonealign_hip.h
+++ b/include/clonealign_hip.h
@@ -73,6 +73,7 @@
   CA_VAR_CELL_LEAN = 1 << 24,
   CA_VAR_MOM_LAST = 1 << 25,
   CA_VAR_CELL_MFMA = 1 << 26,
+  CA_VAR_Y2 = 1 << 27,
   CA_VAR_RIDE_SEQ = 1 << 13
 };
 enum ca_variant_on {
@@ -86,6 +87,7 @@
   CA_VARX_SERIES = 1 << 8,
   CA_VARX_Y4 = 1 << 9,
   CA_VARX_MOM_LAST = 1 << 10,
+  CA_VARX_Y2 = 1 << 11,
   CA_VARX_ASYNC_SMALL = 1 << 1
 };
 #define CA_OPT_VERBOSE 0x80000000u
@@ -144,6 +146,9 @@
   int32_t mom_last;
   int32_t mom_free_slots;
   int32_t cell_mfma;
+  int32_t y_stream_n2;
+  int64_t y_stream_esc;
+  int64_t y_stream_bytes;
 } ca_info;
 enum ca_transport { CA_TRANSPORT_NONE = 0, CA_TRANSPORT_RCCL = 1, CA_TRANSPORT_HOST = 2, CA_TRANSPORT_P2P = 3 };
 
```

Measured after the change: 10000 iterations/s (median of 6 runs). 1.08x the previous value.
